# Wells-Group/pmg-dolfinx

Hardware: NVIDIA B200
Metric: fine-level Gdof/s per p-MG V-cycle (P4->P2->P1, Chebyshev(2), CSR coarse solve) (higher is better)
Workload: dtype f64

## Files before the change

### include/pmgx.h

```cpp
#ifndef PMGX_H
#define PMGX_H

#include <stddef.h>
#include <stdint.h>

#ifdef __cplusplus
extern "C" {
#endif

#define PMGX_OK 0
#define PMGX_ERR_ARG 1
#define PMGX_ERR_CUDA 2
#define PMGX_ERR_NCCL 3
#define PMGX_ERR_NUMERIC 4
#define PMGX_ERR_UNSUPPORTED 5

#define PMGX_MAX_DEGREE 8
#define PMGX_NCCL_ID_BYTES 128

typedef struct pmgx_ctx pmgx_ctx;
typedef struct pmgx_halo pmgx_halo;
typedef struct pmgx_operator pmgx_operator;
typedef struct pmgx_cheb pmgx_cheb;
typedef struct pmgx_cg pmgx_cg;
typedef struct pmgx_interp pmgx_interp;
typedef struct pmgx_coarse pmgx_coarse;
typedef struct pmgx_vcycle pmgx_vcycle;
typedef struct pmgx_boxmesh pmgx_boxmesh;
typedef struct pmgx_ghostmesh pmgx_ghostmesh;
typedef struct pmgx_amg_hier pmgx_amg_hier;

const char* pmgx_last_error_string(void);
int pmgx_version(void);

int pmgx_gll_tables(int degree, double* points_h, double* weights_h, double* dphi_h);
int pmgx_gll_interp_1d(int degree_coarse, int degree_fine, double* interp_h);

int pmgx_tqli(double* d_h, double* e_h, int n);

int pmgx_nccl_unique_id(void* id_h);
int pmgx_ctx_create(int device, int rank, int nranks, const void* nccl_id_h, pmgx_ctx** out);
int pmgx_ctx_destroy(pmgx_ctx* ctx);
int pmgx_ctx_sync(pmgx_ctx* ctx);
void* pmgx_ctx_stream(pmgx_ctx* ctx);
int pmgx_ctx_rank(pmgx_ctx* ctx);
int pmgx_ctx_nranks(pmgx_ctx* ctx);
long long pmgx_ctx_launch_count(pmgx_ctx* ctx);
int pmgx_ctx_uses_p2p(pmgx_ctx* ctx);
int pmgx_ctx_profile(pmgx_ctx* ctx, int on);
int pmgx_ctx_profile_read(pmgx_ctx* ctx, int degree, double* ms_total_h, long long* launches_h);

int pmgx_halo_create(pmgx_ctx* ctx, int n_owned, int n_ghost,
                     int n_send_nbr, const int* send_ranks_h, const int* send_offsets_h,
                     const int32_t* send_idx_h,
                     int n_recv_nbr, const int* recv_ranks_h, const int* recv_offsets_h,
                     const int32_t* recv_idx_h, pmgx_halo** out);
int pmgx_halo_destroy(pmgx_halo* h);
int pmgx_halo_uses_p2p(pmgx_halo* h);
int pmgx_halo_fwd_begin(pmgx_halo* h, double* x);
int pmgx_halo_fwd_end(pmgx_halo* h, double* x);
int pmgx_halo_rev(pmgx_halo* h, double* x);
int pmgx_pack(pmgx_ctx* ctx, int n, const int32_t* idx, const double* in, double* out);
int pmgx_unpack(pmgx_ctx* ctx, int n, const int32_t* idx, const double* in, double* out);
int pmgx_unpack_add(pmgx_ctx* ctx, int n, const int32_t* idx, const double* in, double* out);

int pmgx_vec_set(pmgx_ctx* ctx, double* x, long long n, double v);
int pmgx_vec_copy(pmgx_ctx* ctx, double* a, const double* b, long long n);
int pmgx_vec_axpy(pmgx_ctx* ctx, double* r, double alpha, const double* x,
                  const double* y, long long n);
int pmgx_vec_scale(pmgx_ctx* ctx, double* r, double alpha, long long n);
int pmgx_vec_pointwise_mult(pmgx_ctx* ctx, double* w, const double* x,
                            const double* y, long long n);
int pmgx_vec_mask_bc(pmgx_ctx* ctx, double* b, const int8_t* bc, long long n);
int pmgx_vec_dot(pmgx_ctx* ctx, const double* a, const double* b, long long n, double* result_h);
int pmgx_vec_norm(pmgx_ctx* ctx, const double* a, long long n, int linf, double* result_h);

#define PMGX_LAP_DEFAULT 0
#define PMGX_LAP_LITERAL_DETJ 1
#define PMGX_LAP_NO_DIAG 2
#define PMGX_LAP_STREAM_G 4
#define PMGX_LAP_RECOMPUTE_G 8
#define PMGX_LAP_GEOM_Q2 16

int pmgx_laplacian_create(pmgx_ctx* ctx, int degree, int n_cells, const int32_t* dofmap,
                          const double* xgeom, int n_points, const int32_t* geom_dofmap,
                          const double* kappa, const int32_t* lcells_h, int n_lcells,
                          const int32_t* bcells_h, int n_bcells, const int8_t* bc_marker,
                          int n_owned, int n_ghost, pmgx_halo* halo, int flags,
                          pmgx_operator** out);
int pmgx_laplacian_get_G(pmgx_operator* op, double* G_out);
int pmgx_laplacian_is_affine(pmgx_operator* op);
int pmgx_laplacian_kernel_name(pmgx_operator* op, char* name_h, int cap);
int pmgx_laplacian_device_bytes(pmgx_operator* op, long long* bytes_h);

int pmgx_csr_create(pmgx_ctx* ctx, int n_rows, int n_ghost, const int32_t* row_ptr_h,
                    const int32_t* off_diag_offset_h, const int32_t* cols_h,
                    const double* values_h, pmgx_halo* halo, pmgx_operator** out);
int pmgx_csr_from_laplacian(pmgx_operator* lap, pmgx_operator** out);
long long pmgx_csr_nnz(pmgx_operator* op);
int pmgx_csr_get(pmgx_operator* op, int32_t* row_ptr_h, int32_t* cols_h, double* values_h);

int pmgx_operator_apply(pmgx_operator* op, double* x, double* y);
int pmgx_operator_get_diag_inverse(pmgx_operator* op, double* out);
int pmgx_operator_set_diag_inverse(pmgx_operator* op, const double* in);
int pmgx_operator_n_owned(pmgx_operator* op);
int pmgx_operator_n_ghost(pmgx_operator* op);
int pmgx_operator_destroy(pmgx_operator* op);

int pmgx_cheb_create(pmgx_ctx* ctx, int n_owned, int n_ghost, double eig_min, double eig_max,
                     pmgx_cheb** out);
int pmgx_cheb_set_max_iterations(pmgx_cheb* s, int max_iter);
int pmgx_cheb_solve(pmgx_cheb* s, pmgx_operator* A, double* x, const double* b,
                    double* resid_hist_h);
int pmgx_cheb_residual(pmgx_cheb* s, pmgx_operator* A, double* x, const double* b,
                       double* rnorm_h);
int pmgx_cheb_destroy(pmgx_cheb* s);

int pmgx_cg_create(pmgx_ctx* ctx, int n_owned, int n_ghost, pmgx_cg** out);
int pmgx_cg_set_max_iterations(pmgx_cg* s, int max_iter);
int pmgx_cg_set_tolerance(pmgx_cg* s, double rtol);
int pmgx_cg_store_coefficients(pmgx_cg* s, int on);
int pmgx_cg_set_preconditioner(pmgx_cg* s, pmgx_vcycle* M);
int pmgx_cg_solve(pmgx_cg* s, pmgx_operator* A, double* x, const double* b, int* iters_h);
int pmgx_cg_num_coefficients(pmgx_cg* s);
int pmgx_cg_get_coefficients(pmgx_cg* s, double* alphas_h, double* betas_h, double* residuals_h);
int pmgx_cg_get_history(pmgx_cg* s, double* rnorm0_h, double* rnorms_h, int* n_h);
int pmgx_cg_compute_eigenvalues(pmgx_cg* s, double* eig_h);
int pmgx_cg_destroy(pmgx_cg* s);

int pmgx_interp_create(pmgx_ctx* ctx, int degree_coarse, int degree_fine, int n_cells,
                       const int32_t* dofmap_coarse, const int32_t* dofmap_fine,
                       int n_coarse_total, int n_fine_total,
                       const int32_t* lcells_h, int n_lcells, const int32_t* bcells_h,
                       int n_bcells, pmgx_halo* halo_c, pmgx_halo* halo_f, pmgx_interp** out);
int pmgx_interp_prolong(pmgx_interp* it, double* coarse, double* fine);
int pmgx_interp_restrict(pmgx_interp* it, double* fine, double* coarse);
int pmgx_interp_destroy(pmgx_interp* it);

int pmgx_coarse_create(pmgx_ctx* ctx, pmgx_operator* A_csr, int max_iter, double rtol,
                       pmgx_coarse** out);
int pmgx_coarse_create_amg(pmgx_ctx* ctx, pmgx_operator* A_csr, int max_iter, double rtol, int nu,
                           int min_coarse, int max_levels, pmgx_coarse** out);
int pmgx_coarse_solve(pmgx_coarse* cs, double* x, const double* b, int* iters_h);
int pmgx_coarse_last_iterations(pmgx_coarse* cs);
int pmgx_coarse_last_status(pmgx_coarse* cs, int* converged_h, double* rel_residual_h);
int pmgx_coarse_num_levels(pmgx_coarse* cs);
int pmgx_coarse_level_info(pmgx_coarse* cs, int level, long long* out_h);
int pmgx_coarse_apply_preconditioner(pmgx_coarse* cs, const double* r, double* u);
int pmgx_coarse_destroy(pmgx_coarse* cs);

typedef int (*pmgx_allgather_fn)(void* user, const void* mine, size_t bytes, void* all);
int pmgx_amg_setup_h(int n_rows, const int32_t* row_ptr_h, const int32_t* cols_h, const double* values_h,
                     int min_coarse, int max_levels, pmgx_amg_hier** out);
int pmgx_amg_setup_dist_h(int rank, int nranks, int n_owned, int n_ghost, const int32_t* row_ptr_h,
                          const int32_t* cols_h, const double* values_h, int n_send_nbr, const int* send_ranks_h,
                          const int* send_offsets_h, const int32_t* send_idx_h, int n_recv_nbr,
                          const int* recv_ranks_h, const int* recv_offsets_h, const int32_t* recv_idx_h,
                          pmgx_allgather_fn allgather, void* user, int min_coarse, int max_levels,
                          pmgx_amg_hier** out);
int pmgx_amg_level_dist_sizes(pmgx_amg_hier* h, int level, long long* out_h);
int pmgx_amg_level_get_restriction(pmgx_amg_hier* h, int level, int32_t* r_ptr_h, int32_t* r_cols_h, double* r_vals_h);
int pmgx_amg_level_dist_get(pmgx_amg_hier* h, int level, int* ghost_src_h, int32_t* ghost_rid_h, int* send_ranks_h,
                            int* send_offsets_h, int32_t* send_idx_h, int* recv_ranks_h, int* recv_offsets_h,
                            int32_t* recv_idx_h, double* inv_rows_h);
int pmgx_csr_drop_zeros_h(int n_rows, const int32_t* ptr_h, const int32_t* cols_h, const double* vals_h,
                          int32_t* out_ptr_h, int32_t* out_cols_h, double* out_vals_h, long long* kept_h);
int pmgx_amg_num_levels(pmgx_amg_hier* h);
int pmgx_amg_level_sizes(pmgx_amg_hier* h, int level, long long* out_h);
int pmgx_amg_level_get(pmgx_amg_hier* h, int level, int32_t* a_ptr_h, int32_t* a_cols_h, double* a_vals_h,
                       int32_t* p_ptr_h, int32_t* p_cols_h, double* p_vals_h, double* lmax_h);
int pmgx_amg_destroy(pmgx_amg_hier* h);

#define PMGX_VC_DEFAULT 0
#define PMGX_VC_LITERAL_REFERENCE_BC 1
#define PMGX_VC_DIAGNOSTICS 2
#define PMGX_VC_LITERAL_SEQUENCE 4
int pmgx_vcycle_create(pmgx_ctx* ctx, int n_levels, pmgx_operator** ops, pmgx_cheb** smoothers,
                       pmgx_interp** interps, const int8_t** bc_markers, pmgx_coarse* coarse,
                       int flags, pmgx_vcycle** out);
int pmgx_vcycle_apply(pmgx_vcycle* vc, const double* b, double* u, double* rnorm_h);
int pmgx_vcycle_get_diagnostics(pmgx_vcycle* vc, double* out_h, int cap, int* n_h);
int pmgx_vcycle_destroy(pmgx_vcycle* vc);

int pmgx_boxmesh_create(int nx, int ny, int nz, int px, int py, int pz, int rank,
                        double perturb, uint64_t seed, pmgx_boxmesh** out);
int pmgx_boxmesh_destroy(pmgx_boxmesh* m);
int pmgx_boxmesh_sizes(pmgx_boxmesh* m, long long* out_h);
int pmgx_boxmesh_geometry(pmgx_boxmesh* m, double* xgeom_h, int32_t* geom_dofmap_h);
int pmgx_boxmesh_cell_lists(pmgx_boxmesh* m, int32_t* lcells_h, int32_t* bcells_h);
int pmgx_boxmesh_space_sizes(pmgx_boxmesh* m, int degree, long long* out_h);
int pmgx_boxmesh_space(pmgx_boxmesh* m, int degree, int32_t* dofmap_h, int8_t* bc_h,
                       long long* l2g_h, double* coords_h);
int pmgx_boxmesh_halo_lists(pmgx_boxmesh* m, int degree, int* send_ranks_h, int* send_offsets_h,
                            int32_t* send_idx_h, int* recv_ranks_h, int* recv_offsets_h,
                            int32_t* recv_idx_h);
int pmgx_boxmesh_fit(long long ndofs_total, int order, int* nxyz_h);

int pmgx_ghostmesh_create(int rank, int nranks, long long n_cells, const long long* cell_vertices_h,
                          const int* cell_owner_h, long long n_vertices, const double* coords_h,
                          pmgx_ghostmesh** out);
int pmgx_ghostmesh_create_q2(int rank, int nranks, long long n_cells, const long long* cell_nodes_h,
                             const int* cell_owner_h, long long n_nodes, const double* coords_h,
                             pmgx_ghostmesh** out);
int pmgx_ghostmesh_nodes_per_cell(pmgx_ghostmesh* m);
int pmgx_ghostmesh_destroy(pmgx_ghostmesh* m);
int pmgx_ghostmesh_sizes(pmgx_ghostmesh* m, long long* out_h);
int pmgx_ghostmesh_geometry(pmgx_ghostmesh* m, double* xgeom_h, int32_t* geom_dofmap_h, long long* cell_gid_h);
int pmgx_ghostmesh_cell_lists(pmgx_ghostmesh* m, int32_t* lcells_h, int32_t* bcells_h);
int pmgx_ghostmesh_space_sizes(pmgx_ghostmesh* m, int degree, long long* out_h);
int pmgx_ghostmesh_space(pmgx_ghostmesh* m, int degree, int32_t* dofmap_h, int8_t* bc_h, long long* l2g_h,
                         double* coords_h);
int pmgx_ghostmesh_halo_lists(pmgx_ghostmesh* m, int degree, int* send_ranks_h, int* send_offsets_h,
                              int32_t* send_idx_h, int* recv_ranks_h, int* recv_offsets_h, int32_t* recv_idx_h);

int pmgx_laplacian_rhs(pmgx_operator* lap, const double* fvals, double g, double* b);
int pmgx_bc_marker_exterior(pmgx_ctx* ctx, int degree, int n_cells, const int32_t* geom_dofmap,
                            const int32_t* dofmap, int n_owned, int n_ghost, pmgx_halo* halo, int8_t* marker_out);

int pmgx_laplacian_lift(pmgx_operator* lap, const double* gvals, double* b);

#ifdef __cplusplus
}
#endif
#endif
```

### pmg_dolfinx_b200/api.py

```python
import ctypes
import numpy as np
import torch

from .capi import lib, check, ptr, PmgxError


LAP_DEFAULT = 0
LAP_LITERAL_DETJ = 1
LAP_NO_DIAG = 2
LAP_STREAM_G = 4
LAP_RECOMPUTE_G = 8
LAP_GEOM_Q2 = 16

Q2_CORNERS = (0, 2, 6, 8, 18, 20, 24, 26)


def corner_columns(geometry_dofmap):
    g = geometry_dofmap.reshape(-1, 27)[:, list(Q2_CORNERS)]
    return g.contiguous() if isinstance(g, torch.Tensor) else np.ascontiguousarray(g)


def _np(a, dtype):
    return np.ascontiguousarray(a, dtype=dtype)


class Context:

    def __init__(self, device=0, rank=0, nranks=1, nccl_id=None):
        h = ctypes.c_void_p()
        idp = None
        if nccl_id is not None:
            self._id = (ctypes.c_char * 128).from_buffer_copy(bytes(nccl_id))
            idp = ctypes.addressof(self._id)
        check(lib.pmgx_ctx_create(device, rank, nranks, idp, ctypes.addressof(h)))
        self.h = h
        self.device = torch.device("cuda", device)
        self.rank, self.nranks = rank, nranks
        self.stream = torch.cuda.ExternalStream(lib.pmgx_ctx_stream(self.h), device=self.device)
        torch.cuda.set_device(self.device)
        torch.cuda.set_stream(self.stream)

    @staticmethod
    def nccl_unique_id():
        buf = (ctypes.c_char * 128)()
        check(lib.pmgx_nccl_unique_id(ctypes.addressof(buf)))
        return bytes(buf)

    def sync(self):
        check(lib.pmgx_ctx_sync(self.h))

    def launch_count(self):
        return int(lib.pmgx_ctx_launch_count(self.h))

    def zeros(self, n, dtype=torch.float64):
        return torch.zeros(int(n), dtype=dtype, device=self.device)

    def to_device(self, a, dtype=None):
        t = torch.as_tensor(np.ascontiguousarray(a))
        if dtype is not None:
            t = t.to(dtype)
        return t.to(self.device)

    def close(self):
        if self.h:
            check(lib.pmgx_ctx_destroy(self.h))
            self.h = None


def gll_tables(degree):
    n = degree + 1
    x, w, D = np.zeros(n), np.zeros(n), np.zeros(n * n)
    check(lib.pmgx_gll_tables(degree, ptr(x), ptr(w), ptr(D)))
    return x, w, D.reshape(n, n)


def gll_interp_1d(pc, pf):
    M = np.zeros((pf + 1) * (pc + 1))
    check(lib.pmgx_gll_interp_1d(pc, pf, ptr(M)))
    return M.reshape(pf + 1, pc + 1)


def exterior_bc_marker(ctx, degree, geometry_dofmap, dofmap, n_owned, n_ghost=0, halo=None):
    out = torch.zeros(int(n_owned) + int(n_ghost), dtype=torch.int8, device=ctx.device)
    n_cells = int(geometry_dofmap.numel() // 8)
    check(lib.pmgx_bc_marker_exterior(ctx.h, degree, n_cells, ptr(geometry_dofmap), ptr(dofmap), int(n_owned), int(n_ghost),
                                      halo.h if halo is not None else None, ptr(out)))
    return out


def tqli(d, e):
    d = _np(d, np.float64).copy()
    e = _np(e, np.float64).copy()
    check(lib.pmgx_tqli(ptr(d), ptr(e), len(d)))
    return d


def boxmesh_fit(ndofs_total, order):
    out = np.zeros(3, dtype=np.int32)
    check(lib.pmgx_boxmesh_fit(int(ndofs_total), order, ptr(out)))
    return tuple(int(v) for v in out)


class BoxMesh:

    def __init__(self, n, pgrid=(1, 1, 1), rank=0, perturb=0.0, seed=1234):
        h = ctypes.c_void_p()
        check(lib.pmgx_boxmesh_create(n[0], n[1], n[2], pgrid[0], pgrid[1], pgrid[2], rank,
                                      float(perturb), seed, ctypes.addressof(h)))
        self.h = h
        self.n, self.pgrid, self.rank = tuple(n), tuple(pgrid), rank
        s = np.zeros(5, dtype=np.int64)
        check(lib.pmgx_boxmesh_sizes(self.h, ptr(s)))
        self.n_cells, self.n_owned_cells, self.n_points, nl, nb = (int(v) for v in s)
        self.xgeom = np.zeros((self.n_points, 3))
        self.geom_dofmap = np.zeros((self.n_cells, 8), dtype=np.int32)
        check(lib.pmgx_boxmesh_geometry(self.h, ptr(self.xgeom), ptr(self.geom_dofmap)))
        self.lcells = np.zeros(nl, dtype=np.int32)
        self.bcells = np.zeros(nb, dtype=np.int32)
        check(lib.pmgx_boxmesh_cell_lists(self.h, ptr(self.lcells), ptr(self.bcells)))

    def space(self, degree, want_coords=False):
        s = np.zeros(7, dtype=np.int64)
        check(lib.pmgx_boxmesh_space_sizes(self.h, degree, ptr(s)))
        sp = HostSpace()
        sp.degree = degree
        (sp.n_owned, sp.n_ghost, nsn, nst, nrn, nrt, sp.n_global) = (int(v) for v in s)
        nd3 = (degree + 1) ** 3
        nt = sp.n_owned + sp.n_ghost
        sp.dofmap = np.zeros((self.n_cells, nd3), dtype=np.int32)
        sp.bc = np.zeros(nt, dtype=np.int8)
        sp.l2g = np.zeros(nt, dtype=np.int64)
        sp.coords = np.zeros((nt, 3)) if want_coords else None
        check(lib.pmgx_boxmesh_space(self.h, degree, ptr(sp.dofmap), ptr(sp.bc), ptr(sp.l2g),
                                     ptr(sp.coords)))
        sp.send_ranks = np.zeros(nsn, dtype=np.int32)
        sp.send_offsets = np.zeros(nsn + 1, dtype=np.int32)
        sp.send_idx = np.zeros(nst, dtype=np.int32)
        sp.recv_ranks = np.zeros(nrn, dtype=np.int32)
        sp.recv_offsets = np.zeros(nrn + 1, dtype=np.int32)
        sp.recv_idx = np.zeros(nrt, dtype=np.int32)
        check(lib.pmgx_boxmesh_halo_lists(self.h, degree, ptr(sp.send_ranks), ptr(sp.send_offsets),
                                          ptr(sp.send_idx), ptr(sp.recv_ranks), ptr(sp.recv_offsets),
                                          ptr(sp.recv_idx)))
        return sp

    def close(self):
        if self.h:
            lib.pmgx_boxmesh_destroy(self.h)
            self.h = None


class HostSpace:
    pass


class GhostLayerMesh:

    def __init__(self, cell_vertices, cell_owner, coords, rank=0, nranks=1):
        cv = _np(cell_vertices, np.int64)
        npc = 27 if cv.ndim == 2 and cv.shape[1] == 27 else 8
        cv = cv.reshape(-1, npc)
        ow = _np(cell_owner, np.int32)
        xs = _np(coords, np.float64).reshape(-1, 3)
        h = ctypes.c_void_p()
        create = lib.pmgx_ghostmesh_create_q2 if npc == 27 else lib.pmgx_ghostmesh_create
        check(create(rank, nranks, len(cv), ptr(cv), ptr(ow), len(xs), ptr(xs), ctypes.addressof(h)))
        self.h, self.rank, self.nranks = h, rank, nranks
        self.nodes_per_cell = int(lib.pmgx_ghostmesh_nodes_per_cell(self.h))
        s = np.zeros(5, dtype=np.int64)
        check(lib.pmgx_ghostmesh_sizes(self.h, ptr(s)))
        self.n_cells, self.n_owned_cells, self.n_points, nl, nb = (int(v) for v in s)
        self.xgeom = np.zeros((self.n_points, 3))
        self.geom_dofmap = np.zeros((self.n_cells, self.nodes_per_cell), dtype=np.int32)
        self.cell_gid = np.zeros(self.n_cells, dtype=np.int64)
        check(lib.pmgx_ghostmesh_geometry(self.h, ptr(self.xgeom), ptr(self.geom_dofmap), ptr(self.cell_gid)))
        self.lcells = np.zeros(nl, dtype=np.int32)
        self.bcells = np.zeros(nb, dtype=np.int32)
        check(lib.pmgx_ghostmesh_cell_lists(self.h, ptr(self.lcells), ptr(self.bcells)))

    def space(self, degree, want_coords=True):
        s = np.zeros(7, dtype=np.int64)
        check(lib.pmgx_ghostmesh_space_sizes(self.h, degree, ptr(s)))
        sp = HostSpace()
        sp.degree = degree
        (sp.n_owned, sp.n_ghost, nsn, nst, nrn, nrt, sp.n_global) = (int(v) for v in s)
        nt = sp.n_owned + sp.n_ghost
        sp.dofmap = np.zeros((self.n_cells, (degree + 1) ** 3), dtype=np.int32)
        sp.bc = np.zeros(nt, dtype=np.int8)
        sp.l2g = np.zeros(nt, dtype=np.int64)
        sp.coords = np.zeros((nt, 3)) if want_coords else None
        check(lib.pmgx_ghostmesh_space(self.h, degree, ptr(sp.dofmap), ptr(sp.bc), ptr(sp.l2g), ptr(sp.coords)))
        sp.send_ranks = np.zeros(nsn, dtype=np.int32)
        sp.send_offsets = np.zeros(nsn + 1, dtype=np.int32)
        sp.send_idx = np.zeros(nst, dtype=np.int32)
        sp.recv_ranks = np.zeros(nrn, dtype=np.int32)
        sp.recv_offsets = np.zeros(nrn + 1, dtype=np.int32)
        sp.recv_idx = np.zeros(nrt, dtype=np.int32)
        check(lib.pmgx_ghostmesh_halo_lists(self.h, degree, ptr(sp.send_ranks), ptr(sp.send_offsets), ptr(sp.send_idx),
                                            ptr(sp.recv_ranks), ptr(sp.recv_offsets), ptr(sp.recv_idx)))
        return sp

    def close(self):
        if self.h:
            lib.pmgx_ghostmesh_destroy(self.h)
            self.h = None


class Halo:

    def __init__(self, ctx, n_owned, n_ghost, send_ranks=(), send_offsets=(0,), send_idx=(),
                 recv_ranks=(), recv_offsets=(0,), recv_idx=()):
        self.ctx, self.n_owned, self.n_ghost = ctx, int(n_owned), int(n_ghost)
        sr, so, si = _np(send_ranks, np.int32), _np(send_offsets, np.int32), _np(send_idx, np.int32)
        rr, ro, ri = _np(recv_ranks, np.int32), _np(recv_offsets, np.int32), _np(recv_idx, np.int32)
        h = ctypes.c_void_p()
        check(lib.pmgx_halo_create(ctx.h, self.n_owned, self.n_ghost, len(sr), ptr(sr), ptr(so), ptr(si),
                                   len(rr), ptr(rr), ptr(ro), ptr(ri), ctypes.addressof(h)))
        self.h = h

    @classmethod
    def from_space(cls, ctx, sp):
        return cls(ctx, sp.n_owned, sp.n_ghost, sp.send_ranks, sp.send_offsets, sp.send_idx,
                   sp.recv_ranks, sp.recv_offsets, sp.recv_idx)


class Vector:

    def __init__(self, ctx, n_owned, n_ghost=0, halo=None):
        self.ctx, self.n_owned, self.n_ghost, self.halo = ctx, int(n_owned), int(n_ghost), halo
        self.data = ctx.zeros(self.n_owned + self.n_ghost)

    @property
    def size_local(self):
        return self.n_owned

    def set(self, v):
        check(lib.pmgx_vec_set(self.ctx.h, ptr(self.data), self.n_owned + self.n_ghost, float(v)))

    def copy_from_host(self, a):
        a = _np(a, np.float64)
        self.data[: self.n_owned].copy_(torch.from_numpy(a[: self.n_owned]))

    def array(self):
        return self.data

    def mutable_array(self):
        return self.data

    def data_copy(self):
        self.ctx.sync()
        return self.data.cpu().numpy()

    def scatter_fwd_begin(self):
        if self.halo is not None:
            check(lib.pmgx_halo_fwd_begin(self.halo.h, ptr(self.data)))

    def scatter_fwd_end(self):
        if self.halo is not None:
            check(lib.pmgx_halo_fwd_end(self.halo.h, ptr(self.data)))

    def scatter_fwd(self):
        self.scatter_fwd_begin()
        self.scatter_fwd_end()

    def scatter_rev(self):
        if self.halo is not None:
            check(lib.pmgx_halo_rev(self.halo.h, ptr(self.data)))


def _same(a, b):
    if a.n_owned != b.n_owned:
        raise PmgxError(1, "Incompatible vector sizes")


def inner_product(a, b):
    _same(a, b)
    r = ctypes.c_double()
    check(lib.pmgx_vec_dot(a.ctx.h, ptr(a.data), ptr(b.data), a.n_owned, ctypes.addressof(r)))
    return r.value


def squared_norm(a):
    return inner_product(a, a)


def norm(a, kind="l2"):
    if kind not in ("l2", "linf"):
        raise PmgxError(1, "Norm type not supported")
    r = ctypes.c_double()
    check(lib.pmgx_vec_norm(a.ctx.h, ptr(a.data), a.n_owned, 1 if kind == "linf" else 0, ctypes.addressof(r)))
    return r.value


def axpy(r, alpha, x, y):
    check(lib.pmgx_vec_axpy(r.ctx.h, ptr(r.data), float(alpha), ptr(x.data), ptr(y.data), x.n_owned))


def scale(r, alpha):
    check(lib.pmgx_vec_scale(r.ctx.h, ptr(r.data), float(alpha), r.n_owned + r.n_ghost))


def copy(a, b):
    check(lib.pmgx_vec_copy(a.ctx.h, ptr(a.data), ptr(b.data), a.n_owned))


def pointwise_mult(w, x, y):
    check(lib.pmgx_vec_pointwise_mult(w.ctx.h, ptr(w.data), ptr(x.data), ptr(y.data), x.n_owned))


class _Operator:
    h = None

    def __call__(self, x, y):
        check(lib.pmgx_operator_apply(self.h, ptr(x.data), ptr(y.data)))

    def get_diag_inverse(self, v):
        check(lib.pmgx_operator_get_diag_inverse(self.h, ptr(v.data)))

    def set_diag_inverse(self, v):
        check(lib.pmgx_operator_set_diag_inverse(self.h, ptr(v.data)))

    @property
    def n_owned(self):
        return lib.pmgx_operator_n_owned(self.h)

    @property
    def n_ghost(self):
        return lib.pmgx_operator_n_ghost(self.h)

    def destroy(self):
        if self.h:
            check(lib.pmgx_operator_destroy(self.h))
            self.h = None


class MatFreeLaplacian(_Operator):

    def __init__(self, ctx, degree, coefficients, dofmap, xgeom, geometry_dofmap, lcells, bcells,
                 bc_marker, n_owned, n_ghost=0, halo=None, flags=0):
        self.ctx, self.degree = ctx, degree
        self._keep = (coefficients, dofmap, xgeom, geometry_dofmap, bc_marker, halo)
        lc, bc_ = _np(lcells, np.int32), _np(bcells, np.int32)
        n_cells = int(dofmap.numel() // ((degree + 1) ** 3)) if degree >= 0 else 0
        h = ctypes.c_void_p()
        check(lib.pmgx_laplacian_create(
            ctx.h, degree, n_cells, ptr(dofmap), ptr(xgeom), int(xgeom.numel() // 3), ptr(geometry_dofmap),
            ptr(coefficients), ptr(lc), len(lc), ptr(bc_), len(bc_), ptr(bc_marker), int(n_owned),
            int(n_ghost), halo.h if halo is not None else None, flags, ctypes.addressof(h)))
        self.h = h
        self.n_list = len(lc) + len(bc_)

    def is_affine(self):
        return bool(lib.pmgx_laplacian_is_affine(self.h))

    def device_bytes(self):
        b = ctypes.c_longlong()
        check(lib.pmgx_laplacian_device_bytes(self.h, ctypes.addressof(b)))
        return b.value

    def kernel_name(self):
        buf = ctypes.create_string_buffer(96)
        check(lib.pmgx_laplacian_kernel_name(self.h, ctypes.addressof(buf), 96))
        return buf.value.decode()

    def geometry_factors(self):
        nq = (self.degree + 1) ** 3
        G = self.ctx.zeros(self.n_list * nq * 6)
        check(lib.pmgx_laplacian_get_G(self.h, ptr(G)))
        self.ctx.sync()
        return G.cpu().numpy().reshape(self.n_list, nq, 6)

    def assemble_rhs(self, fvals, g, b):
        check(lib.pmgx_laplacian_rhs(self.h, ptr(fvals), float(g), ptr(b.data)))

    def lift(self, gvals, b):
        check(lib.pmgx_laplacian_lift(self.h, ptr(gvals), ptr(b.data)))

    def to_csr(self):
        return MatrixOperator._from_handle(self.ctx, lambda out: lib.pmgx_csr_from_laplacian(self.h, out))


class MatrixOperator(_Operator):

    def __init__(self, ctx, row_ptr, off_diag_offset, cols, values, n_ghost=0, halo=None):
        self.ctx = ctx
        rp, od = _np(row_ptr, np.int32), _np(off_diag_offset, np.int32)
        co, va = _np(cols, np.int32), _np(values, np.float64)
        h = ctypes.c_void_p()
        check(lib.pmgx_csr_create(ctx.h, len(rp) - 1, int(n_ghost), ptr(rp), ptr(od), ptr(co), ptr(va),
                                  halo.h if halo is not None else None, ctypes.addressof(h)))
        self.h = h

    @classmethod
    def _from_handle(cls, ctx, make):
        self = cls.__new__(cls)
        self.ctx = ctx
        h = ctypes.c_void_p()
        check(make(ctypes.addressof(h)))
        self.h = h
        return self

    def nnz(self):
        return int(lib.pmgx_csr_nnz(self.h))

    def to_host(self):
        n = self.n_owned
        rp = np.zeros(n + 1, dtype=np.int32)
        co = np.zeros(self.nnz(), dtype=np.int32)
        va = np.zeros(self.nnz())
        check(lib.pmgx_csr_get(self.h, ptr(rp), ptr(co), ptr(va)))
        return rp, co, va


class Chebyshev:

    def __init__(self, ctx, n_owned, n_ghost, eig_range):
        self.ctx = ctx
        h = ctypes.c_void_p()
        check(lib.pmgx_cheb_create(ctx.h, int(n_owned), int(n_ghost), float(eig_range[0]), float(eig_range[1]),
                                   ctypes.addressof(h)))
        self.h = h
        self.max_iter = 0

    def set_max_iterations(self, n):
        self.max_iter = int(n)
        check(lib.pmgx_cheb_set_max_iterations(self.h, int(n)))

    def solve(self, A, x, b, verbose=False):
        hist = np.zeros(self.max_iter + 1) if verbose else None
        check(lib.pmgx_cheb_solve(self.h, A.h, ptr(x.data), ptr(b.data), ptr(hist)))
        return hist

    def residual(self, A, x, b):
        r = ctypes.c_double()
        check(lib.pmgx_cheb_residual(self.h, A.h, ptr(x.data), ptr(b.data), ctypes.addressof(r)))
        return r.value


class CGSolver:

    def __init__(self, ctx, n_owned, n_ghost=0):
        self.ctx = ctx
        h = ctypes.c_void_p()
        check(lib.pmgx_cg_create(ctx.h, int(n_owned), int(n_ghost), ctypes.addressof(h)))
        self.h = h

    def set_max_iterations(self, n):
        check(lib.pmgx_cg_set_max_iterations(self.h, int(n)))

    def set_tolerance(self, rtol):
        check(lib.pmgx_cg_set_tolerance(self.h, float(rtol)))

    def store_coefficients(self, on):
        check(lib.pmgx_cg_store_coefficients(self.h, 1 if on else 0))

    def set_preconditioner(self, pmg):
        if pmg is not None and pmg.h is None:
            pmg._build()
        self._pmg = pmg
        check(lib.pmgx_cg_set_preconditioner(self.h, pmg.h if pmg is not None else None))

    def solve(self, A, x, b, verbose=False):
        k = ctypes.c_int()
        check(lib.pmgx_cg_solve(self.h, A.h, ptr(x.data), ptr(b.data), ctypes.addressof(k)))
        return k.value

    def _coeffs(self):
        n = lib.pmgx_cg_num_coefficients(self.h)
        a, b, r = np.zeros(n), np.zeros(n), np.zeros(n)
        check(lib.pmgx_cg_get_coefficients(self.h, ptr(a), ptr(b), ptr(r)))
        return a, b, r

    def alphas(self):
        return self._coeffs()[0]

    def betas(self):
        return self._coeffs()[1]

    def residual(self):
        return self._coeffs()[2][-1]

    def history(self, cap=4096):
        r0, n = ctypes.c_double(), ctypes.c_int()
        h = np.zeros(cap)
        check(lib.pmgx_cg_get_history(self.h, ctypes.addressof(r0), ptr(h), ctypes.addressof(n)))
        return r0.value, h[: n.value].copy()

    def compute_eigenvalues(self):
        n = lib.pmgx_cg_num_coefficients(self.h)
        e = np.zeros(max(n, 1))
        check(lib.pmgx_cg_compute_eigenvalues(self.h, ptr(e)))
        return e[:n]


class Interpolator:

    def __init__(self, ctx, degree_coarse, degree_fine, Q1_dofmap, Q2_dofmap, n_coarse_total, n_fine_total,
                 l_cells, b_cells, halo_coarse=None, halo_fine=None):
        self.ctx = ctx
        self._keep = (Q1_dofmap, Q2_dofmap, halo_coarse, halo_fine)
        lc, bc_ = _np(l_cells, np.int32), _np(b_cells, np.int32)
        n_cells = int(Q1_dofmap.numel() // ((degree_coarse + 1) ** 3))
        h = ctypes.c_void_p()
        check(lib.pmgx_interp_create(ctx.h, degree_coarse, degree_fine, n_cells, ptr(Q1_dofmap), ptr(Q2_dofmap),
                                     int(n_coarse_total), int(n_fine_total), ptr(lc), len(lc), ptr(bc_), len(bc_),
                                     halo_coarse.h if halo_coarse is not None else None,
                                     halo_fine.h if halo_fine is not None else None, ctypes.addressof(h)))
        self.h = h

    def interpolate(self, Q1_vector, Q2_vector):
        check(lib.pmgx_interp_prolong(self.h, ptr(Q1_vector.data), ptr(Q2_vector.data)))

    def reverse_interpolate(self, Q2_vector, Q1_vector):
        check(lib.pmgx_interp_restrict(self.h, ptr(Q2_vector.data), ptr(Q1_vector.data)))


class CoarseSolverType:

    def __init__(self, ctx, A_csr, max_iter=60, rtol=1e-5, amg=True, nu=2, min_coarse=0, max_levels=0):
        self.ctx, self.A, self.amg = ctx, A_csr, bool(amg)
        h = ctypes.c_void_p()
        if amg:
            check(lib.pmgx_coarse_create_amg(ctx.h, A_csr.h, int(max_iter), float(rtol), int(nu), int(min_coarse),
                                             int(max_levels), ctypes.addressof(h)))
        else:
            check(lib.pmgx_coarse_create(ctx.h, A_csr.h, int(max_iter), float(rtol), ctypes.addressof(h)))
        self.h = h

    def solve(self, x, b):
        k = ctypes.c_int()
        check(lib.pmgx_coarse_solve(self.h, ptr(x.data), ptr(b.data), ctypes.addressof(k)))
        return k.value

    def last_iterations(self):
        return int(lib.pmgx_coarse_last_iterations(self.h))

    def last_status(self):
        c, r = ctypes.c_int(), ctypes.c_double()
        check(lib.pmgx_coarse_last_status(self.h, ctypes.addressof(c), ctypes.addressof(r)))
        return bool(c.value), r.value

    def levels(self):
        out = []
        for l in range(lib.pmgx_coarse_num_levels(self.h)):
            v = np.zeros(5, dtype=np.int64)
            check(lib.pmgx_coarse_level_info(self.h, l, ptr(v)))
            out.append(tuple(int(t) for t in v))
        return out

    def apply_preconditioner(self, r, u):
        check(lib.pmgx_coarse_apply_preconditioner(self.h, ptr(r.data), ptr(u.data)))


class MultigridPreconditioner:

    def __init__(self, ctx, bc_markers, flags=0):
        self.ctx, self.bc_markers, self.flags = ctx, list(bc_markers), flags
        self.solvers = self.operators = self.interpolators = None
        self.coarse_solver = None
        self.h = None

    def set_solvers(self, s):
        self.solvers = list(s)

    def set_coarse_solver(self, s):
        self.coarse_solver = s

    def set_operators(self, o):
        self.operators = list(o)

    def set_interpolators(self, i):
        self.interpolators = list(i)

    def _build(self):
        nl = len(self.operators)
        P = ctypes.c_void_p * nl
        ops = P(*[o.h for o in self.operators])
        sm = P(*[s.h for s in self.solvers])
        bcs = P(*[ptr(b) for b in self.bc_markers])
        its = (ctypes.c_void_p * max(nl - 1, 1))(*[i.h for i in (self.interpolators or [])])
        h = ctypes.c_void_p()
        check(lib.pmgx_vcycle_create(self.ctx.h, nl, ctypes.addressof(ops), ctypes.addressof(sm),
                                     ctypes.addressof(its), ctypes.addressof(bcs),
                                     self.coarse_solver.h if self.coarse_solver is not None else None,
                                     self.flags, ctypes.addressof(h)))
        self.h = h

    def apply(self, x, y, verbose=False):
        if self.h is None:
            self._build()
        r = ctypes.c_double()
        check(lib.pmgx_vcycle_apply(self.h, ptr(x.data), ptr(y.data), ctypes.addressof(r) if verbose else None))
        return r.value if verbose else None

    def diagnostics(self, cap=256):
        out, n = np.zeros(cap), ctypes.c_int()
        check(lib.pmgx_vcycle_get_diagnostics(self.h, ptr(out), cap, ctypes.addressof(n)))
        return out[: n.value].copy()
```

### pmg_dolfinx_b200/csrc/amg.cu

```cuda
#include "common.hpp"
#include "operator.hpp"
#include "csr.hpp"
#include "solvers.hpp"
#include "amg.hpp"

#include <algorithm>
#include <cstdlib>
#include <cstring>

namespace pmgx
{
namespace
{
__global__ void __launch_bounds__(256)
k_dense_rows(int n_rows, int n_cols, const double* __restrict__ inv, const double* __restrict__ b,
             double* __restrict__ x)
{
  const int row = (blockIdx.x * blockDim.x + threadIdx.x) >> 5, lane = threadIdx.x & 31;
  if (row >= n_rows)
    return;
  const double* r = inv + (size_t)row * n_cols;
  double s = 0.0;
  for (int c = lane; c < n_cols; c += 32)
    s = fma(r[c], b[c], s);
#pragma unroll
  for (int o = 16; o > 0; o >>= 1)
    s += __shfl_xor_sync(0xffffffffu, s, o);
  if (lane == 0)
    x[row] = s;
}

__global__ void k_permute(int n, const int32_t* __restrict__ perm, const double* __restrict__ in, double* __restrict__ out)
{
  const int g = blockIdx.x * blockDim.x + threadIdx.x;
  if (g < n)
    out[g] = in[perm[g]];
}

struct RectSell
{
  int n_rows = 0;
  DevBuf<long long> slice_ptr;
  DevBuf<int32_t> cols;
  DevBuf<double> vals;
  void upload(const amg::Csr& M, cudaStream_t st)
  {
    n_rows = M.n_rows;
    const int ns = (n_rows + 31) / 32;
    std::vector<long long> sp((size_t)ns + 1, 0);
    for (int s = 0; s < ns; ++s)
    {
      int w = 0;
      for (int r = s * 32; r < std::min(n_rows, s * 32 + 32); ++r)
        w = std::max(w, (int)(M.ptr[r + 1] - M.ptr[r]));
      sp[s + 1] = sp[s] + (long long)w * 32;
    }
    std::vector<int32_t> c((size_t)std::max<long long>(sp[ns], 1), 0);
    std::vector<double> v((size_t)std::max<long long>(sp[ns], 1), 0.0);
    for (int r = 0; r < n_rows; ++r)
      for (int32_t j = M.ptr[r], k = 0; j < M.ptr[r + 1]; ++j, ++k)
      {
        const size_t p = (size_t)sp[r >> 5] + (size_t)k * 32 + (r & 31);
        c[p] = M.cols[j];
        v[p] = M.vals[j];
      }
    slice_ptr.upload(sp.data(), sp.size(), st);
    cols.upload(c.data(), c.size(), st);
    vals.upload(v.data(), v.size(), st);
  }
};

struct RectCsr
{
  int n_rows = 0;
  DevBuf<int32_t> ptr, cols;
  DevBuf<double> vals;
  void upload(const amg::Csr& M, cudaStream_t st)
  {
    n_rows = M.n_rows;
    ptr.upload(M.ptr.data(), M.ptr.size(), st);
    cols.upload(M.cols.data(), M.cols.size(), st);
    vals.upload(M.vals.data(), M.vals.size(), st);
  }
};

pmgx_halo* make_halo(pmgx_ctx* c, int n_owned, int n_ghost, const amg::Plan& p)
{
  if (c->nranks == 1)
    return nullptr;
  pmgx_halo* h = nullptr;
  const int rc = pmgx_halo_create(c, n_owned, n_ghost, (int)p.send_ranks.size(), p.send_ranks.data(), p.send_offsets.data(),
                                  p.send_idx.data(), (int)p.recv_ranks.size(), p.recv_ranks.data(), p.recv_offsets.data(),
                                  p.recv_idx.data(), &h);
  if (rc != PMGX_OK)
    throw Error{rc};
  static const bool ss = !(getenv("PMGX_AMG_SINGLE_STREAM") && atoi(getenv("PMGX_AMG_SINGLE_STREAM")) == 0);
  h->single_stream = ss && h->p2p && h->n_send() + h->n_recv() <= 65536;
  return h;
}

struct AmgPrecond : Precond
{
  struct Lv
  {
    int n_owned = 0, n_ghost = 0;
    long long nnz = 0;
    pmgx_operator* A = nullptr;
    bool own_A = false;
    pmgx_operator* A_lp = nullptr;
    pmgx_halo* halo = nullptr;
    pmgx_halo* halo_v = nullptr;
    pmgx_cheb* sm = nullptr;
    RectCsr R;
    RectSell P;
    DevBuf<double> x, b;
    DevBuf<double> x2, r2;
    long long nnz_p = 0;
    bool dense = false;
    int n_global = 0;
    DevBuf<double> inv;
    pmgx_halo* gather = nullptr;
    bool repl_first = false;
    int n_mine = 0;
    pmgx_halo* repl_gather = nullptr;
    DevBuf<double> bg;
    DevBuf<int32_t> perm;
  };
  pmgx_ctx* ctx = nullptr;
  std::vector<Lv> lv;
  int nu = 2;
  int gamma = 1;
  int gamma_from = 0;

  ~AmgPrecond() override
  {
    for (Lv& L : lv)
    {
      if (L.sm)
        pmgx_cheb_destroy(L.sm);
      if (L.A_lp)
        pmgx_operator_destroy(L.A_lp);
      if (L.own_A && L.A)
        pmgx_operator_destroy(L.A);
      if (L.halo)
        pmgx_halo_destroy(L.halo);
      if (L.gather)
        pmgx_halo_destroy(L.gather);
      if (L.repl_gather)
        pmgx_halo_destroy(L.repl_gather);
    }
  }

  void cycle(int l, const double* b, double* x)
  {
    Lv& L = lv[l];
    if (l + 1 == (int)lv.size())
    {
      if (L.dense)
      {
        double* bb = L.b.p;
        if (b != bb)
          vec::copy(ctx, bb, b, L.n_owned);
        if (L.gather)
        {
          halo_fwd_begin(L.gather, bb);
          halo_fwd_end(L.gather, bb);
        }
        if (L.n_owned > 0)
        {
          k_dense_rows<<<(L.n_owned * 32 + 255) / 256, 256, 0, ctx->stream>>>(L.n_owned, L.n_global, L.inv.p, bb, x);
          check_launch("k_dense_rows");
          count_launch(ctx);
        }
      }
      else
        cheb_solve(L.sm, L.A, x, b, nullptr, true, CHEB_R_NONE);
      return;
    }
    Lv& C = lv[l + 1];
    pmgx_operator* As = L.A_lp ? L.A_lp : L.A;
    cheb_solve(L.sm, As, x, b, nullptr, true, CHEB_R_FULL);
    if (L.halo_v)
    {
      halo_fwd_begin(L.halo_v, L.sm->r.p);
      halo_fwd_end(L.halo_v, L.sm->r.p);
    }
    if (C.repl_first)
    {
      spmv_rect(ctx, C.n_mine, L.R.ptr.p, L.R.cols.p, L.R.vals.p, L.sm->r.p, C.bg.p, false, 32);
      halo_fwd_begin(C.repl_gather, C.bg.p);
      halo_fwd_end(C.repl_gather, C.bg.p);
      k_permute<<<(C.n_owned + 255) / 256, 256, 0, ctx->stream>>>(C.n_owned, C.perm.p, C.bg.p, C.b.p);
      check_launch("k_permute");
      count_launch(ctx);
    }
    else
      spmv_rect(ctx, C.n_owned, L.R.ptr.p, L.R.cols.p, L.R.vals.p, L.sm->r.p, C.b.p, false, 32);
    cycle(l + 1, C.b.p, C.x.p);
    if (gamma == 2 && l >= gamma_from && l + 2 < (int)lv.size())
    {
      C.A->apply(C.x.p, C.r2.p);
      vec::axpy(ctx, C.r2.p, -1.0, C.r2.p, C.b.p, C.n_owned);
      cycle(l + 1, C.r2.p, C.x2.p);
      vec::axpy(ctx, C.x.p, 1.0, C.x2.p, C.x.p, C.n_owned);
    }
    if (C.halo_v)
    {
      halo_fwd_begin(C.halo_v, C.x.p);
      halo_fwd_end(C.halo_v, C.x.p);
    }
    spmv_sell_rect(ctx, L.n_owned, L.P.slice_ptr.p, L.P.cols.p, L.P.vals.p, C.x.p, x, true);
    cheb_solve(L.sm, As, x, b, nullptr, false, CHEB_R_NONE);
  }

  void apply(const double* r, double* u) override { cycle(0, r, u); }
};

amg::Plan plan_of(pmgx_halo* h)
{
  amg::Plan p;
  if (!h)
    return p;
  p.send_ranks = h->send_ranks;
  p.send_offsets = h->send_offsets;
  p.recv_ranks = h->recv_ranks;
  p.recv_offsets = h->recv_offsets;
  if (p.send_offsets.empty())
    p.send_offsets.assign(1, 0);
  if (p.recv_offsets.empty())
    p.recv_offsets.assign(1, 0);
  p.send_idx.resize((size_t)h->n_send());
  p.recv_idx.resize((size_t)h->n_recv());
  if (!p.send_idx.empty())
    PMGX_CUDA(cudaMemcpy(p.send_idx.data(), h->send_idx.p, p.send_idx.size() * sizeof(int32_t), cudaMemcpyDeviceToHost));
  if (!p.recv_idx.empty())
    PMGX_CUDA(cudaMemcpy(p.recv_idx.data(), h->recv_idx.p, p.recv_idx.size() * sizeof(int32_t), cudaMemcpyDeviceToHost));
  return p;
}
}
}

using pmgx::AmgPrecond;

extern "C"
{
int pmgx_coarse_create_amg(pmgx_ctx* ctx, pmgx_operator* A, int max_iter, double rtol, int nu, int min_coarse,
                           int max_levels, pmgx_coarse** out)
{
  PMGX_API_BEGIN
  PMGX_REQUIRE(ctx && A && out && max_iter >= 0, "coarse_create_amg: bad arguments");
  PMGX_REQUIRE(A->kind == pmgx_operator::CSR, "coarse_create_amg: the operator must be an assembled CSR operator");
  PMGX_REQUIRE(nu >= 1 && nu <= 8, "coarse_create_amg: nu must be in 1..8");
  PMGX_CUDA(cudaSetDevice(ctx->device));
  if (min_coarse <= 0)
    min_coarse = 600;
  if (max_levels <= 0)
    max_levels = 12;
  auto* Ac = static_cast<pmgx::CsrOperator*>(A);
  PMGX_REQUIRE(ctx->nranks == 1 || Ac->halo || Ac->n_ghost == 0, "coarse_create_amg: the operator has ghosts but no halo");
  pmgx::amg::Csr A0;
  A0.ptr.resize((size_t)Ac->n_owned + 1);
  A0.cols.resize((size_t)Ac->nnz);
  A0.vals.resize((size_t)Ac->nnz);
  {
    const int rc = pmgx_csr_get(A, A0.ptr.data(), A0.cols.data(), A0.vals.data());
    if (rc != PMGX_OK)
      return rc;
    std::vector<std::pair<int32_t, double>> row;
    for (int i = 0; i < Ac->n_owned; ++i)
    {
      bool sorted = true;
      for (int32_t j = A0.ptr[i] + 1; j < A0.ptr[i + 1] && sorted; ++j)
        sorted = A0.cols[j - 1] < A0.cols[j];
      if (sorted)
        continue;
      row.clear();
      for (int32_t j = A0.ptr[i]; j < A0.ptr[i + 1]; ++j)
        row.emplace_back(A0.cols[j], A0.vals[j]);
      std::sort(row.begin(), row.end());
      for (size_t t = 0; t < row.size(); ++t)
        A0.cols[A0.ptr[i] + t] = row[t].first, A0.vals[A0.ptr[i] + t] = row[t].second;
    }
  }
  pmgx::amg::Csr Az;
  if (Ac->n_owned > 0)
  {
    A0.n_rows = Ac->n_owned;
    A0.n_cols = Ac->n_owned + Ac->n_ghost;
    Az = pmgx::amg::drop_stored_zeros(A0);
    if (Az.nnz() * 5 > A0.nnz() * 4)
      Az = pmgx::amg::Csr();
  }
  const pmgx::amg::Plan plan0 = pmgx::plan_of(Ac->halo);
  pmgx::amg::Comm cm;
  cm.rank = ctx->rank;
  cm.nranks = ctx->nranks;
  cm.allgather = [ctx](const void* mine, size_t bytes, void* all)
  {
    std::vector<char> buf;
    pmgx::p2p::allgather_bytes(ctx, mine, bytes, buf);
    std::memcpy(all, buf.data(), bytes * (size_t)ctx->nranks);
  };
  pmgx::amg::Hierarchy H;
  pmgx::amg::setup(H, std::move(A0), Ac->n_owned, Ac->n_ghost, plan0, cm, min_coarse, max_levels);

  std::unique_ptr<AmgPrecond> M(new AmgPrecond());
  M->ctx = ctx;
  M->nu = nu;
  int nu_coarse = nu;
  if (const char* e = getenv("PMGX_AMG_NU_COARSE"))
    nu_coarse = std::min(std::max(atoi(e), 1), 8);
  if (const char* e = getenv("PMGX_AMG_GAMMA"))
    M->gamma = atoi(e) == 2 ? 2 : 1;
  if (const char* e = getenv("PMGX_AMG_GAMMA_FROM"))
    M->gamma_from = std::max(atoi(e), 0);
  const bool use_lp = !(getenv("PMGX_AMG_LP") && atoi(getenv("PMGX_AMG_LP")) == 0);
  const int fuse_from = getenv("PMGX_AMG_FUSE_FROM") ? atoi(getenv("PMGX_AMG_FUSE_FROM")) : 0;
  const int nl = (int)H.levels.size();
  M->lv.resize((size_t)nl);
  for (int l = 0; l < nl; ++l)
  {
    pmgx::amg::Level& L = H.levels[l];
    AmgPrecond::Lv& D = M->lv[l];
    D.n_owned = L.n_owned;
    D.n_ghost = L.n_ghost;
    D.nnz = L.A.nnz();
    const bool last = l + 1 == nl;
    if (l == 0)
    {
      D.A = A;
      D.halo_v = Ac->halo;
      if (!Az.ptr.empty())
      {
        std::vector<int32_t> off((size_t)Ac->n_owned);
        for (int i = 0; i < Ac->n_owned; ++i)
        {
          int32_t j = Az.ptr[i];
          while (j < Az.ptr[i + 1] && Az.cols[j] < Ac->n_owned)
            ++j;
          off[i] = j;
        }
        pmgx_operator* Acmp = nullptr;
        const int rc = pmgx_csr_create(ctx, Ac->n_owned, Ac->n_ghost, Az.ptr.data(), off.data(), Az.cols.data(),
                                       Az.vals.data(), Ac->halo, &Acmp);
        if (rc != PMGX_OK)
          return rc;
        D.A = Acmp;
        D.own_A = true;
      }
    }
    else
    {
      if (!L.replicated)
      {
        D.halo = pmgx::make_halo(ctx, L.n_owned, L.n_ghost, L.plan);
        D.halo_v = D.halo;
      }
      else if (L.n_mine > 0 || !L.gather_perm.empty())
      {
        D.repl_first = true;
        D.n_mine = L.n_mine;
        D.repl_gather = pmgx::make_halo(ctx, L.n_mine, L.n_owned - L.n_mine, L.repl_plan);
        D.bg.alloc((size_t)std::max(L.n_owned, 1));
        PMGX_CUDA(cudaMemsetAsync(D.bg.p, 0, (size_t)std::max(L.n_owned, 1) * sizeof(double), ctx->stream));
        D.perm.upload(L.gather_perm.data(), L.gather_perm.size(), ctx->stream);
      }
      std::vector<int32_t> off((size_t)L.n_owned);
      for (int i = 0; i < L.n_owned; ++i)
      {
        int32_t j = L.A.ptr[i];
        while (j < L.A.ptr[i + 1] && L.A.cols[j] < L.n_owned)
          ++j;
        off[i] = j;
      }
      const int rc = pmgx_csr_create(ctx, L.n_owned, L.n_ghost, L.A.ptr.data(), off.data(), L.A.cols.data(),
                                     L.A.vals.data(), D.halo, &D.A);
      if (rc != PMGX_OK)
        return rc;
      D.own_A = true;
      const size_t nt = (size_t)L.n_owned + L.n_ghost;
      for (auto* buf : {&D.x, &D.b, &D.x2, &D.r2})
      {
        buf->alloc(nt);
        if (nt > 0)
          PMGX_CUDA(cudaMemsetAsync(buf->p, 0, nt * sizeof(double), ctx->stream));
      }
    }
    {
      const int rc = pmgx_cheb_create(ctx, L.n_owned, L.n_ghost, 0.1 * L.lmax, L.lmax, &D.sm);
      if (rc != PMGX_OK)
        return rc;
      D.sm->max_iter = (last && !L.dense) ? 4 * nu : (l == 0 ? nu : nu_coarse);
      D.sm->fuse = l >= fuse_from;
    }
    if (l == 0 && !last && use_lp)
      D.A_lp = pmgx::make_lp(static_cast<pmgx::CsrOperator*>(D.A));
    D.nnz_p = L.P.nnz();
    if (!last)
    {
      D.P.upload(pmgx::amg::drop_stored_zeros(L.P), ctx->stream);
      D.R.upload(pmgx::amg::drop_stored_zeros(L.R), ctx->stream);
    }
    else if (L.dense)
    {
      D.dense = true;
      D.n_global = (int)L.n_global;
      D.inv.upload(L.inv_rows.data(), L.inv_rows.size(), ctx->stream);
      const int n_gather = (int)L.n_global - L.n_owned;
      if (!L.replicated)
        D.gather = pmgx::make_halo(ctx, L.n_owned, n_gather, L.gather_plan);
      const size_t nt = (size_t)L.n_owned + std::max(L.n_ghost, n_gather);
      D.b.alloc(nt);
      if (nt > 0)
        PMGX_CUDA(cudaMemsetAsync(D.b.p, 0, nt * sizeof(double), ctx->stream));
    }
  }
  PMGX_CUDA(cudaStreamSynchronize(ctx->stream));

  pmgx_coarse* cs = nullptr;
  const int rc = pmgx_coarse_create(ctx, M->lv[0].A, max_iter, rtol, &cs);
  if (rc != PMGX_OK)
    return rc;
  cs->M = M.release();
  cs->check_every = 1;
  if (const char* e = getenv("PMGX_COARSE_CHECK_EVERY"))
    cs->check_every = std::max(atoi(e), 1);
  *out = cs;
  PMGX_API_END
}

int pmgx_coarse_num_levels(pmgx_coarse* cs)
{
  if (!cs)
    return -1;
  return cs->M ? (int)static_cast<AmgPrecond*>(cs->M)->lv.size() : 1;
}

int pmgx_coarse_level_info(pmgx_coarse* cs, int level, long long* out_h)
{
  PMGX_API_BEGIN
  PMGX_REQUIRE(cs && out_h && level >= 0 && level < pmgx_coarse_num_levels(cs), "coarse_level_info: bad arguments");
  if (!cs->M)
  {
    out_h[0] = cs->A->n_owned;
    out_h[1] = pmgx_csr_nnz(cs->A);
    out_h[2] = cs->A->n_ghost;
    out_h[3] = 0;
    out_h[4] = 0;
  }
  else
  {
    const AmgPrecond::Lv& L = static_cast<AmgPrecond*>(cs->M)->lv[level];
    out_h[0] = L.n_owned;
    out_h[1] = L.nnz;
    out_h[2] = L.n_ghost;
    out_h[3] = L.dense ? 1 : 0;
    out_h[4] = L.nnz_p;
  }
  PMGX_API_END
}

int pmgx_coarse_apply_preconditioner(pmgx_coarse* cs, const double* r, double* u)
{
  PMGX_API_BEGIN
  PMGX_REQUIRE(cs && r && u && r != u, "coarse_apply_preconditioner: bad arguments");
  PMGX_CUDA(cudaSetDevice(cs->ctx->device));
  if (cs->M)
    cs->M->apply(r, u);
  else
    pmgx::vec::pointwise_mult(cs->ctx, u, r, cs->A->diag_inv.p, cs->A->n_owned);
  PMGX_API_END
}
}
```

### pmg_dolfinx_b200/csrc/common.hpp

```cpp
#pragma once

#include <cuda_runtime.h>
#include <nccl.h>

#include <cstdarg>
#include <cstdint>
#include <cstdio>
#include <memory>
#include <algorithm>
#include <stdexcept>
#include <string>
#include <utility>
#include <vector>

#include "../../include/pmgx.h"

namespace pmgx
{
void set_error(const char* fmt, ...);

struct Error
{
  int code;
};

#define PMGX_CUDA(call)                                                                            \
  do                                                                                               \
  {                                                                                                \
    cudaError_t _e = (call);                                                                       \
    if (_e != cudaSuccess)                                                                         \
    {                                                                                              \
      pmgx::set_error("%s:%d CUDA error: %s (%s)", __FILE__, __LINE__, cudaGetErrorString(_e),     \
                      #call);                                                                      \
      throw pmgx::Error{PMGX_ERR_CUDA};                                                            \
    }                                                                                              \
  } while (0)

#define PMGX_NCCL(call)                                                                            \
  do                                                                                               \
  {                                                                                                \
    ncclResult_t _e = (call);                                                                      \
    if (_e != ncclSuccess)                                                                         \
    {                                                                                              \
      pmgx::set_error("%s:%d NCCL error: %s (%s)", __FILE__, __LINE__, ncclGetErrorString(_e),     \
                      #call);                                                                      \
      throw pmgx::Error{PMGX_ERR_NCCL};                                                            \
    }                                                                                              \
  } while (0)

#define PMGX_REQUIRE(cond, ...)                                                                    \
  do                                                                                               \
  {                                                                                                \
    if (!(cond))                                                                                   \
    {                                                                                              \
      pmgx::set_error(__VA_ARGS__);                                                                \
      throw pmgx::Error{PMGX_ERR_ARG};                                                             \
    }                                                                                              \
  } while (0)

#define PMGX_API_BEGIN try {
#define PMGX_API_END                                                                               \
  }                                                                                                \
  catch (const pmgx::Error& e) { return e.code; }                                                  \
  catch (const std::exception& e)                                                                  \
  {                                                                                                \
    pmgx::set_error("exception: %s", e.what());                                                    \
    return PMGX_ERR_ARG;                                                                           \
  }                                                                                                \
  return PMGX_OK;

template <typename T>
struct DevBuf
{
  T* p = nullptr;
  size_t n = 0;
  DevBuf() = default;
  DevBuf(const DevBuf&) = delete;
  DevBuf& operator=(const DevBuf&) = delete;
  DevBuf(DevBuf&& o) noexcept : p(o.p), n(o.n)
  {
    o.p = nullptr;
    o.n = 0;
  }
  ~DevBuf() { release(); }
  void alloc(size_t count)
  {
    release();
    n = count;
    if (count > 0)
      PMGX_CUDA(cudaMalloc(&p, count * sizeof(T)));
  }
  void release()
  {
    if (p)
      cudaFree(p);
    p = nullptr;
    n = 0;
  }
  void upload(const T* h, size_t count, cudaStream_t s)
  {
    alloc(count);
    if (count > 0)
    {
      PMGX_CUDA(cudaMemcpyAsync(p, h, count * sizeof(T), cudaMemcpyHostToDevice, s));
      PMGX_CUDA(cudaStreamSynchronize(s));
    }
  }
};
}

struct pmgx_ctx
{
  int device = 0;
  int rank = 0;
  int nranks = 1;
  int num_sms = 148;
  cudaStream_t stream = nullptr;
  cudaStream_t comm_stream = nullptr;
  ncclComm_t comm = nullptr;
  double* d_scalars = nullptr;
  double* h_scalars = nullptr;
  double* h_scalars_dev = nullptr;
  unsigned int* d_counter = nullptr;
  double* d_partials = nullptr;
  int max_red_blocks = 0;
  bool p2p = false;
  double* ar_local = nullptr;
  double** d_ar_peers = nullptr;
  std::vector<void*> p2p_mapped;
  unsigned long long* d_ar_epoch = nullptr;
  unsigned long long p2p_timeout_ns = 600ull * 1000000000ull;
  long long launches = 0;
  bool profiling = false;
  std::vector<std::pair<cudaEvent_t, cudaEvent_t>> prof[PMGX_MAX_DEGREE + 1];
};

namespace pmgx
{
inline void count_launch(pmgx_ctx* ctx, int n = 1) { ctx->launches += n; }
inline void check_launch(const char* what)
{
  cudaError_t e = cudaGetLastError();
  if (e != cudaSuccess)
  {
    set_error("kernel launch failed (%s): %s", what, cudaGetErrorString(e));
    throw Error{PMGX_ERR_CUDA};
  }
}

void gll_points_weights(int n, std::vector<double>& x, std::vector<double>& w);
void gll_deriv_matrix(const std::vector<double>& x, std::vector<double>& D);
void gll_interp_matrix(int pc, int pf, std::vector<double>& M);

namespace p2p
{
void allgather_bytes(pmgx_ctx* c, const void* mine, size_t bytes, std::vector<char>& all);
bool all_agree(pmgx_ctx* c, bool mine);
void ctx_setup(pmgx_ctx* c);
void ctx_teardown(pmgx_ctx* c);
void allreduce(pmgx_ctx* c, int slot, int count, bool is_max);
}

namespace vec
{
void set(pmgx_ctx* c, double* x, long long n, double v);
void copy(pmgx_ctx* c, double* a, const double* b, long long n);
void axpy(pmgx_ctx* c, double* r, double alpha, const double* x, const double* y, long long n);
void scale(pmgx_ctx* c, double* r, double alpha, long long n);
void pointwise_mult(pmgx_ctx* c, double* w, const double* x, const double* y, long long n);
void mask_bc(pmgx_ctx* c, double* b, const int8_t* bc, long long n);
void allreduce_scalars(pmgx_ctx* c, int slot, int count, bool is_max);
void dot_device(pmgx_ctx* c, const double* a, const double* b, long long n, int slot);
double read_scalar(pmgx_ctx* c, int slot);
void publish_scalars(pmgx_ctx* c, int slot, int count);
double dot(pmgx_ctx* c, const double* a, const double* b, long long n);
double norm_linf(pmgx_ctx* c, const double* a, long long n);
}
}
```

### pmg_dolfinx_b200/csrc/csr.cu

```cuda
#include "common.hpp"
#include "operator.hpp"
#include "csr.hpp"
#include "solvers.hpp"

namespace pmgx
{
namespace
{
constexpr int LPR = 8;
constexpr int ST = 256;

constexpr int UNR = 4;
template <bool ACCUM>
__global__ void __launch_bounds__(ST)
k_spmv(int n_rows, const double* __restrict__ vals, const int32_t* __restrict__ beg,
       const int32_t* __restrict__ end, const int32_t* __restrict__ cols,
       const double* __restrict__ x, double* __restrict__ y)
{
  const int gt = blockIdx.x * blockDim.x + threadIdx.x;
  const int row = gt / LPR, lane = gt % LPR;
  double s = 0.0;
  if (row < n_rows)
  {
    const int e = end[row];
    for (int j0 = beg[row] + lane; j0 < e; j0 += UNR * LPR)
    {
      int c[UNR];
      double v[UNR];
#pragma unroll
      for (int t = 0; t < UNR; ++t)
      {
        const int jj = j0 + t * LPR;
        const bool ok = jj < e;
        c[t] = ok ? __ldcs(cols + jj) : -1;
        v[t] = ok ? __ldcs(vals + jj) : 0.0;
      }
#pragma unroll
      for (int t = 0; t < UNR; ++t)
        if (c[t] >= 0)
          s = fma(v[t], x[c[t]], s);
    }
  }
#pragma unroll
  for (int o = LPR / 2; o > 0; o >>= 1)
    s += __shfl_xor_sync(0xffffffffu, s, o);
  if (row < n_rows && lane == 0)
    y[row] = ACCUM ? y[row] + s : s;
}

__global__ void __launch_bounds__(ST)
k_spmv_ghost_rows(int n_list, const int32_t* __restrict__ rows, const double* __restrict__ vals,
                  const int32_t* __restrict__ off_diag, const int32_t* __restrict__ row_ptr,
                  const int32_t* __restrict__ cols, const double* __restrict__ x, double* __restrict__ y)
{
  const int gt = blockIdx.x * blockDim.x + threadIdx.x;
  const int li = gt / LPR, lane = gt % LPR;
  double s = 0.0;
  int row = -1;
  if (li < n_list)
  {
    row = rows[li];
    const int e = row_ptr[row + 1];
    for (int j = off_diag[row] + lane; j < e; j += LPR)
      s = fma(vals[j], x[cols[j]], s);
  }
#pragma unroll
  for (int o = LPR / 2; o > 0; o >>= 1)
    s += __shfl_xor_sync(0xffffffffu, s, o);
  if (row >= 0 && lane == 0)
    y[row] += s;
}

template <int MODE>
__device__ __forceinline__ void cheb_row(int i, double q, const double* __restrict__ in, const ChebEp& e)
{
  if (MODE == ChebEp::INIT)
  {
    const double rv = q * (-1.0) + e.b[i];
    e.r[i] = rv;
    e.z_out[i] = (rv * e.dinv[i]) * e.c0;
  }
  else if (MODE == ChebEp::LAST)
    e.r[i] = q * (-1.0) + e.r[i];
  else
  {
    const double rv = q * (-1.0) + e.r[i];
    const double zo = in[i];
    const double zs = zo * e.c1;
    const double zv = (rv * e.dinv[i]) * e.c2 + zs;
    if (MODE == ChebEp::STEP)
    {
      e.r[i] = rv;
      e.z_out[i] = zv;
    }
    const double xo = e.defer == 2 ? zo : (e.defer == 1 ? zo * 1.0 + e.x[i] : e.x[i]);
    e.x[i] = zv * 1.0 + xo;
  }
}

template <typename VT, bool D16, int MODE>
__global__ void __launch_bounds__(ST)
k_spmv_cheb(int n_rows, const VT* __restrict__ vals, const int32_t* __restrict__ beg, const int32_t* __restrict__ end,
            const int32_t* __restrict__ row_ptr, const int16_t* __restrict__ dcol, const int32_t* __restrict__ cols,
            const double* __restrict__ x, const ChebEp e)
{
  const int gt = blockIdx.x * blockDim.x + threadIdx.x;
  const int row = gt / LPR, lane = gt % LPR;
  double s = 0.0;
  if (row < n_rows)
  {
    const int en = end[row];
    for (int j0 = beg[row] + lane; j0 < en; j0 += UNR * LPR)
    {
      int c[UNR];
      VT v[UNR];
#pragma unroll
      for (int t = 0; t < UNR; ++t)
      {
        const int jj = j0 + t * LPR;
        const bool ok = jj < en;
        c[t] = ok ? (D16 ? row + (int)__ldcs(dcol + jj) : __ldcs(cols + jj)) : -1;
        v[t] = ok ? __ldcs(vals + jj) : VT(0);
      }
#pragma unroll
      for (int t = 0; t < UNR; ++t)
        if (c[t] >= 0)
          s = fma((double)v[t], x[c[t]], s);
    }
  }
#pragma unroll
  for (int o = LPR / 2; o > 0; o >>= 1)
    s += __shfl_xor_sync(0xffffffffu, s, o);
  __shared__ double sq[ST / LPR];
  if (lane == 0)
    sq[threadIdx.x / LPR] = s;
  __syncthreads();
  if (threadIdx.x < ST / LPR)
  {
    const int r = blockIdx.x * (ST / LPR) + threadIdx.x;
    if (r < n_rows)
    {
      if (end[r] < row_ptr[r + 1])
        e.scratch[r] = sq[threadIdx.x];
      else
        cheb_row<MODE>(r, sq[threadIdx.x], x, e);
    }
  }
}

template <int MODE>
__global__ void __launch_bounds__(ST)
k_spmv_cheb_ghost_rows(int n_list, const int32_t* __restrict__ rows, const double* __restrict__ vals,
                       const int32_t* __restrict__ off_diag, const int32_t* __restrict__ row_ptr,
                       const int32_t* __restrict__ cols, const double* __restrict__ x, const ChebEp e)
{
  const int gt = blockIdx.x * blockDim.x + threadIdx.x;
  const int li = gt / LPR, lane = gt % LPR;
  double s = 0.0;
  int row = -1;
  if (li < n_list)
  {
    row = rows[li];
    const int en = row_ptr[row + 1];
    for (int j = off_diag[row] + lane; j < en; j += LPR)
      s = fma(vals[j], x[cols[j]], s);
  }
#pragma unroll
  for (int o = LPR / 2; o > 0; o >>= 1)
    s += __shfl_xor_sync(0xffffffffu, s, o);
  if (row >= 0 && lane == 0)
    cheb_row<MODE>(row, e.scratch[row] + s, x, e);
}

template <typename VT, bool D16>
void launch_spmv_cheb(pmgx_ctx* c, int grid, int n_rows, const VT* vals, const int32_t* beg, const int32_t* end,
                      const int32_t* row_ptr, const int16_t* dcol, const int32_t* cols, const double* x, const ChebEp& e)
{
  switch (e.mode)
  {
  case ChebEp::INIT: k_spmv_cheb<VT, D16, ChebEp::INIT><<<grid, ST, 0, c->stream>>>(n_rows, vals, beg, end, row_ptr, dcol, cols, x, e); break;
  case ChebEp::STEP: k_spmv_cheb<VT, D16, ChebEp::STEP><<<grid, ST, 0, c->stream>>>(n_rows, vals, beg, end, row_ptr, dcol, cols, x, e); break;
  case ChebEp::LAST: k_spmv_cheb<VT, D16, ChebEp::LAST><<<grid, ST, 0, c->stream>>>(n_rows, vals, beg, end, row_ptr, dcol, cols, x, e); break;
  default: k_spmv_cheb<VT, D16, ChebEp::XONLY><<<grid, ST, 0, c->stream>>>(n_rows, vals, beg, end, row_ptr, dcol, cols, x, e); break;
  }
  check_launch("k_spmv_cheb");
  count_launch(c);
}

void launch_ghost_rows_cheb(const CsrOperator* A, const double* x, const ChebEp& e)
{
  pmgx_ctx* c = A->ctx;
  const int g2 = (int)(((long long)A->n_ghost_rows * LPR + ST - 1) / ST);
#define PMGX_GR(M)                                                                                                     \
  k_spmv_cheb_ghost_rows<M><<<g2, ST, 0, c->stream>>>(A->n_ghost_rows, A->ghost_rows.p, A->values.p, A->off_diag.p,    \
                                                      A->row_ptr.p, A->cols.p, x, e)
  switch (e.mode)
  {
  case ChebEp::INIT: PMGX_GR(ChebEp::INIT); break;
  case ChebEp::STEP: PMGX_GR(ChebEp::STEP); break;
  case ChebEp::LAST: PMGX_GR(ChebEp::LAST); break;
  default: PMGX_GR(ChebEp::XONLY); break;
  }
#undef PMGX_GR
  check_launch("k_spmv_cheb_ghost_rows");
  count_launch(c);
}

__global__ void k_flag_ghost_rows(int n_rows, const int32_t* __restrict__ off_diag,
                                  const int32_t* __restrict__ row_ptr, int32_t* __restrict__ count,
                                  int32_t* __restrict__ list)
{
  const int i = blockIdx.x * blockDim.x + threadIdx.x;
  if (i < n_rows && off_diag[i] < row_ptr[i + 1])
    list[atomicAdd(count, 1)] = i;
}

__global__ void k_extract_diag_inv(int n_rows, const double* __restrict__ vals,
                                   const int32_t* __restrict__ row_ptr,
                                   const int32_t* __restrict__ cols, double* __restrict__ dinv)
{
  const int i = blockIdx.x * blockDim.x + threadIdx.x;
  if (i >= n_rows)
    return;
  double d = 0.0;
  for (int j = row_ptr[i]; j < row_ptr[i + 1]; ++j)
    if (cols[j] == i)
      d = 1.0 / vals[j];
  dinv[i] = d;
}

constexpr int SLICE = 32;

template <bool D16>
__device__ __forceinline__ double sell_row(int row, int n_rows, const long long* __restrict__ slice_ptr,
                                           const float* __restrict__ vals, const int16_t* __restrict__ dcol,
                                           const int32_t* __restrict__ cols, const double* __restrict__ x)
{
  const int s = row >> 5, lane = row & 31;
  const long long b = slice_ptr[s];
  const int w = (int)((slice_ptr[s + 1] - b) >> 5);
  const float* v = vals + b + lane;
  const int16_t* d = dcol + b + lane;
  const int32_t* c = cols + b + lane;
  const int r = row < n_rows ? row : n_rows - 1;
  double s0 = 0.0, s1 = 0.0;
  int k = 0;
  for (; k + 4 <= w; k += 4)
  {
    float vv[4];
    int cc[4];
#pragma unroll
    for (int t = 0; t < 4; ++t)
    {
      vv[t] = __ldcs(v + (k + t) * SLICE);
      cc[t] = D16 ? r + (int)__ldcs(d + (k + t) * SLICE) : __ldcs(c + (k + t) * SLICE);
    }
    s0 = fma((double)vv[0], x[cc[0]], s0);
    s1 = fma((double)vv[1], x[cc[1]], s1);
    s0 = fma((double)vv[2], x[cc[2]], s0);
    s1 = fma((double)vv[3], x[cc[3]], s1);
  }
  for (; k < w; ++k)
  {
    const float vv = __ldcs(v + k * SLICE);
    const int cc = D16 ? r + (int)__ldcs(d + k * SLICE) : __ldcs(c + k * SLICE);
    s0 = fma((double)vv, x[cc], s0);
  }
  return s0 + s1;
}

template <bool D16>
__global__ void __launch_bounds__(ST)
k_spmv_sell(int n_rows, const long long* __restrict__ slice_ptr, const float* __restrict__ vals,
            const int16_t* __restrict__ dcol, const int32_t* __restrict__ cols, const double* __restrict__ x,
            double* __restrict__ y)
{
  const int row = blockIdx.x * blockDim.x + threadIdx.x;
  if ((row >> 5) >= (n_rows + SLICE - 1) / SLICE)
    return;
  const double s = sell_row<D16>(row, n_rows, slice_ptr, vals, dcol, cols, x);
  if (row < n_rows)
    y[row] = s;
}

template <bool D16, int MODE>
__global__ void __launch_bounds__(ST)
k_spmv_sell_cheb(int n_rows, const long long* __restrict__ slice_ptr, const float* __restrict__ vals,
                 const int16_t* __restrict__ dcol, const int32_t* __restrict__ cols,
                 const int32_t* __restrict__ off_diag, const int32_t* __restrict__ row_ptr,
                 const double* __restrict__ x, const ChebEp e)
{
  const int row = blockIdx.x * blockDim.x + threadIdx.x;
  if ((row >> 5) >= (n_rows + SLICE - 1) / SLICE)
    return;
  const double s = sell_row<D16>(row, n_rows, slice_ptr, vals, dcol, cols, x);
  if (row >= n_rows)
    return;
  if (off_diag && off_diag[row] < row_ptr[row + 1])
    e.scratch[row] = s;
  else
    cheb_row<MODE>(row, s, x, e);
}

template <bool ACCUM>
__global__ void __launch_bounds__(ST)
k_spmv_sell_rect(int n_rows, const long long* __restrict__ slice_ptr, const double* __restrict__ vals,
                 const int32_t* __restrict__ cols, const double* __restrict__ x, double* __restrict__ y)
{
  const int row = blockIdx.x * blockDim.x + threadIdx.x;
  const int s = row >> 5, lane = row & 31;
  if (row >= n_rows)
    return;
  const long long b = slice_ptr[s];
  const int w = (int)((slice_ptr[s + 1] - b) >> 5);
  const double* v = vals + b + lane;
  const int32_t* c = cols + b + lane;
  double s0 = 0.0, s1 = 0.0;
  int k = 0;
  for (; k + 2 <= w; k += 2)
  {
    const double v0 = __ldcs(v + k * SLICE), v1 = __ldcs(v + (k + 1) * SLICE);
    const int c0 = __ldcs(c + k * SLICE), c1 = __ldcs(c + (k + 1) * SLICE);
    s0 = fma(v0, x[c0], s0);
    s1 = fma(v1, x[c1], s1);
  }
  if (k < w)
    s0 = fma(__ldcs(v + k * SLICE), x[__ldcs(c + k * SLICE)], s0);
  y[row] = ACCUM ? y[row] + (s0 + s1) : s0 + s1;
}

__global__ void k_sell_widths(int n_rows, const int32_t* __restrict__ row_ptr, const int32_t* __restrict__ off_diag,
                              const int32_t* __restrict__ cols, long long* __restrict__ widths, int* __restrict__ overflow)
{
  const int row = blockIdx.x * blockDim.x + threadIdx.x;
  int len = 0;
  bool ovf = false;
  if (row < n_rows)
  {
    len = off_diag[row] - row_ptr[row];
    for (int j = row_ptr[row]; j < off_diag[row]; ++j)
    {
      const int dlt = cols[j] - row;
      ovf = ovf || dlt > 32767 || dlt < -32767;
    }
  }
#pragma unroll
  for (int o = 16; o > 0; o >>= 1)
    len = max(len, __shfl_xor_sync(0xffffffffu, len, o));
  if (__any_sync(0xffffffffu, ovf) && (threadIdx.x & 31) == 0)
    atomicOr(overflow, 1);
  if ((threadIdx.x & 31) == 0 && row < n_rows)
    widths[row >> 5] = (long long)len * SLICE;
}

__global__ void k_sell_fill(int n_rows, const int32_t* __restrict__ row_ptr, const int32_t* __restrict__ off_diag,
                            const int32_t* __restrict__ cols, const double* __restrict__ vals,
                            const long long* __restrict__ slice_ptr, float* __restrict__ v32, int16_t* __restrict__ d16,
                            int32_t* __restrict__ c32)
{
  const int row = blockIdx.x * blockDim.x + threadIdx.x;
  const int s = row >> 5, lane = row & 31;
  if (s >= (n_rows + SLICE - 1) / SLICE)
    return;
  const long long b = slice_ptr[s];
  const int w = (int)((slice_ptr[s + 1] - b) >> 5);
  const int r = row < n_rows ? row : n_rows - 1;
  const int beg = row < n_rows ? row_ptr[row] : 0, len = row < n_rows ? off_diag[row] - row_ptr[row] : 0;
  for (int k = 0; k < w; ++k)
  {
    const long long p = b + (long long)k * SLICE + lane;
    const bool ok = k < len;
    v32[p] = ok ? (float)vals[beg + k] : 0.f;
    const int col = ok ? cols[beg + k] : r;
    if (d16)
      d16[p] = (int16_t)(col - r);
    if (c32)
      c32[p] = col;
  }
}

template <int LANES, bool ACCUM>
__global__ void __launch_bounds__(ST)
k_spmv_rect(int n_rows, const double* __restrict__ vals, const int32_t* __restrict__ ptr,
            const int32_t* __restrict__ cols, const double* __restrict__ x, double* __restrict__ y)
{
  const int gt = blockIdx.x * blockDim.x + threadIdx.x;
  const int row = gt / LANES, lane = gt % LANES;
  double s = 0.0;
  if (row < n_rows)
  {
    const int e = ptr[row + 1];
    for (int j = ptr[row] + lane; j < e; j += LANES)
      s = fma(vals[j], x[cols[j]], s);
  }
#pragma unroll
  for (int o = LANES / 2; o > 0; o >>= 1)
    s += __shfl_xor_sync(0xffffffffu, s, o);
  if (row < n_rows && lane == 0)
    y[row] = ACCUM ? y[row] + s : s;
}
}

void spmv_sell_rect(pmgx_ctx* c, int n_rows, const long long* slice_ptr, const int32_t* cols, const double* vals,
                    const double* x, double* y, bool accumulate)
{
  if (n_rows <= 0)
    return;
  const int grid = (n_rows + ST - 1) / ST;
  if (accumulate)
    k_spmv_sell_rect<true><<<grid, ST, 0, c->stream>>>(n_rows, slice_ptr, vals, cols, x, y);
  else
    k_spmv_sell_rect<false><<<grid, ST, 0, c->stream>>>(n_rows, slice_ptr, vals, cols, x, y);
  check_launch("k_spmv_sell_rect");
  count_launch(c);
}

void spmv_rect(pmgx_ctx* c, int n_rows, const int32_t* row_ptr, const int32_t* cols, const double* vals,
               const double* x, double* y, bool accumulate, int lanes)
{
  if (n_rows <= 0)
    return;
  const int grid = (int)(((long long)n_rows * lanes + ST - 1) / ST);
  if (lanes == 32)
  {
    if (accumulate)
      k_spmv_rect<32, true><<<grid, ST, 0, c->stream>>>(n_rows, vals, row_ptr, cols, x, y);
    else
      k_spmv_rect<32, false><<<grid, ST, 0, c->stream>>>(n_rows, vals, row_ptr, cols, x, y);
  }
  else if (lanes == 4)
  {
    if (accumulate)
      k_spmv_rect<4, true><<<grid, ST, 0, c->stream>>>(n_rows, vals, row_ptr, cols, x, y);
    else
      k_spmv_rect<4, false><<<grid, ST, 0, c->stream>>>(n_rows, vals, row_ptr, cols, x, y);
  }
  else
  {
    if (accumulate)
      k_spmv_rect<8, true><<<grid, ST, 0, c->stream>>>(n_rows, vals, row_ptr, cols, x, y);
    else
      k_spmv_rect<8, false><<<grid, ST, 0, c->stream>>>(n_rows, vals, row_ptr, cols, x, y);
  }
  check_launch("k_spmv_rect");
  count_launch(c);
}

void CsrOperator::apply(double* x, double* y)
{
  cudaSetDevice(ctx->device);
  const int grid = (int)(((long long)n_owned * LPR + ST - 1) / ST);
  if (n_ghost > 0)
    vec::set(ctx, y + n_owned, n_ghost, 0.0);
  if (halo)
    halo_fwd_begin(halo, x);
  if (n_owned > 0)
  {
    k_spmv<false><<<grid, ST, 0, ctx->stream>>>(n_owned, values.p, row_ptr.p, off_diag.p, cols.p, x, y);
    check_launch("k_spmv");
    count_launch(ctx);
  }
  if (halo)
    halo_fwd_end(halo, x);
  if (n_ghost_rows > 0)
  {
    const int g2 = (int)(((long long)n_ghost_rows * LPR + ST - 1) / ST);
    k_spmv_ghost_rows<<<g2, ST, 0, ctx->stream>>>(n_ghost_rows, ghost_rows.p, values.p, off_diag.p, row_ptr.p, cols.p,
                                                  x, y);
    check_launch("k_spmv_ghost_rows");
    count_launch(ctx);
  }
}

bool CsrOperator::apply_cheb(double* in, const ChebEp& e)
{
  cudaSetDevice(ctx->device);
  PMGX_REQUIRE(n_ghost_rows == 0 || e.scratch, "apply_cheb: scratch vector missing");
  const int grid = (int)(((long long)n_owned * LPR + ST - 1) / ST);
  if (halo)
    halo_fwd_begin(halo, in);
  if (n_owned > 0)
    launch_spmv_cheb<double, false>(ctx, grid, n_owned, values.p, row_ptr.p, off_diag.p, row_ptr.p, nullptr, cols.p, in, e);
  if (halo)
    halo_fwd_end(halo, in);
  if (n_ghost_rows > 0)
    launch_ghost_rows_cheb(this, in, e);
  return true;
}

namespace
{
template <bool D16>
void launch_sell_cheb(const CsrOperatorLP* L, const double* x, const ChebEp& e)
{
  const CsrOperator* A = L->src;
  const int grid = (L->n_slices * SLICE + ST - 1) / ST;
  const int32_t* od = A->n_ghost_rows > 0 ? A->off_diag.p : nullptr;
#define PMGX_SC(M)                                                                                                     \
  k_spmv_sell_cheb<D16, M><<<grid, ST, 0, L->ctx->stream>>>(L->n_owned, L->slice_ptr.p, L->vals32.p, L->dcol16.p,       \
                                                            L->cols32.p, od, A->row_ptr.p, x, e)
  switch (e.mode)
  {
  case ChebEp::INIT: PMGX_SC(ChebEp::INIT); break;
  case ChebEp::STEP: PMGX_SC(ChebEp::STEP); break;
  case ChebEp::LAST: PMGX_SC(ChebEp::LAST); break;
  default: PMGX_SC(ChebEp::XONLY); break;
  }
#undef PMGX_SC
  check_launch("k_spmv_sell_cheb");
  count_launch(L->ctx);
}
}

void CsrOperatorLP::apply(double* x, double* y)
{
  cudaSetDevice(ctx->device);
  if (n_ghost > 0)
    vec::set(ctx, y + n_owned, n_ghost, 0.0);
  if (halo)
    halo_fwd_begin(halo, x);
  if (n_owned > 0)
  {
    const int grid = (n_slices * SLICE + ST - 1) / ST;
    if (d16)
      k_spmv_sell<true><<<grid, ST, 0, ctx->stream>>>(n_owned, slice_ptr.p, vals32.p, dcol16.p, nullptr, x, y);
    else
      k_spmv_sell<false><<<grid, ST, 0, ctx->stream>>>(n_owned, slice_ptr.p, vals32.p, nullptr, cols32.p, x, y);
    check_launch("k_spmv_sell");
    count_launch(ctx);
  }
  if (halo)
    halo_fwd_end(halo, x);
  if (src->n_ghost_rows > 0)
  {
    const int g2 = (int)(((long long)src->n_ghost_rows * LPR + ST - 1) / ST);
    k_spmv_ghost_rows<<<g2, ST, 0, ctx->stream>>>(src->n_ghost_rows, src->ghost_rows.p, src->values.p, src->off_diag.p,
                                                  src->row_ptr.p, src->cols.p, x, y);
    check_launch("k_spmv_ghost_rows");
    count_launch(ctx);
  }
}

bool CsrOperatorLP::apply_cheb(double* in, const ChebEp& e)
{
  cudaSetDevice(ctx->device);
  PMGX_REQUIRE(src->n_ghost_rows == 0 || e.scratch, "apply_cheb: scratch vector missing");
  if (halo)
    halo_fwd_begin(halo, in);
  if (n_owned > 0)
  {
    if (d16)
      launch_sell_cheb<true>(this, in, e);
    else
      launch_sell_cheb<false>(this, in, e);
  }
  if (halo)
    halo_fwd_end(halo, in);
  if (src->n_ghost_rows > 0)
    launch_ghost_rows_cheb(src, in, e);
  return true;
}

CsrOperatorLP* make_lp(CsrOperator* A)
{
  pmgx_ctx* c = A->ctx;
  std::unique_ptr<CsrOperatorLP> L(new CsrOperatorLP());
  L->ctx = c;
  L->kind = pmgx_operator::CSR;
  L->n_owned = A->n_owned;
  L->n_ghost = A->n_ghost;
  L->halo = A->halo;
  L->src = A;
  L->diag_inv.alloc((size_t)A->n_owned);
  if (A->n_owned > 0)
    PMGX_CUDA(cudaMemcpyAsync(L->diag_inv.p, A->diag_inv.p, (size_t)A->n_owned * sizeof(double), cudaMemcpyDeviceToDevice, c->stream));
  const int n = A->n_owned;
  L->n_slices = (n + SLICE - 1) / SLICE;
  L->slice_ptr.alloc((size_t)L->n_slices + 1);
  PMGX_CUDA(cudaMemsetAsync(L->slice_ptr.p, 0, ((size_t)L->n_slices + 1) * sizeof(long long), c->stream));
  DevBuf<int> ovf;
  ovf.alloc(1);
  PMGX_CUDA(cudaMemsetAsync(ovf.p, 0, sizeof(int), c->stream));
  long long total = 0;
  if (n > 0)
  {
    k_sell_widths<<<(n + ST - 1) / ST, ST, 0, c->stream>>>(n, A->row_ptr.p, A->off_diag.p, A->cols.p, L->slice_ptr.p + 1, ovf.p);
    check_launch("k_sell_widths");
    std::vector<long long> sp((size_t)L->n_slices + 1, 0);
    PMGX_CUDA(cudaMemcpyAsync(sp.data(), L->slice_ptr.p, sp.size() * sizeof(long long), cudaMemcpyDeviceToHost, c->stream));
    PMGX_CUDA(cudaStreamSynchronize(c->stream));
    for (size_t i = 1; i < sp.size(); ++i)
      sp[i] += sp[i - 1];
    total = sp.back();
    PMGX_CUDA(cudaMemcpyAsync(L->slice_ptr.p, sp.data(), sp.size() * sizeof(long long), cudaMemcpyHostToDevice, c->stream));
    PMGX_CUDA(cudaStreamSynchronize(c->stream));
  }
  int o = 0;
  PMGX_CUDA(cudaMemcpyAsync(&o, ovf.p, sizeof(int), cudaMemcpyDeviceToHost, c->stream));
  PMGX_CUDA(cudaStreamSynchronize(c->stream));
  L->d16 = o == 0;
  const size_t cap = (size_t)std::max<long long>(total, 1);
  L->vals32.alloc(cap);
  if (L->d16)
    L->dcol16.alloc(cap);
  else
    L->cols32.alloc(cap);
  if (n > 0)
  {
    k_sell_fill<<<(L->n_slices * SLICE + ST - 1) / ST, ST, 0, c->stream>>>(n, A->row_ptr.p, A->off_diag.p, A->cols.p, A->values.p,
                                                                         L->slice_ptr.p, L->vals32.p, L->dcol16.p, L->cols32.p);
    check_launch("k_sell_fill");
    PMGX_CUDA(cudaStreamSynchronize(c->stream));
  }
  return L.release();
}

void CsrOperator::finish_setup()
{
  n_ghost_rows = 0;
  if (n_owned > 0 && has_ghost_cols)
  {
    DevBuf<int32_t> count;
    count.alloc(1);
    ghost_rows.alloc((size_t)n_owned);
    PMGX_CUDA(cudaMemsetAsync(count.p, 0, sizeof(int32_t), ctx->stream));
    k_flag_ghost_rows<<<(n_owned + 255) / 256, 256, 0, ctx->stream>>>(n_owned, off_diag.p, row_ptr.p, count.p,
                                                                      ghost_rows.p);
    check_launch("k_flag_ghost_rows");
    PMGX_CUDA(cudaMemcpyAsync(&n_ghost_rows, count.p, sizeof(int32_t), cudaMemcpyDeviceToHost, ctx->stream));
    PMGX_CUDA(cudaStreamSynchronize(ctx->stream));
  }
  diag_inv.alloc((size_t)n_owned);
  if (n_owned > 0)
  {
    k_extract_diag_inv<<<(n_owned + 255) / 256, 256, 0, ctx->stream>>>(n_owned, values.p, row_ptr.p,
                                                                       cols.p, diag_inv.p);
    check_launch("k_extract_diag_inv");
    count_launch(ctx);
    PMGX_CUDA(cudaStreamSynchronize(ctx->stream));
  }
}
}

using pmgx::CsrOperator;

extern "C"
{
int pmgx_csr_create(pmgx_ctx* ctx, int n_rows, int n_ghost, const int32_t* row_ptr_h,
                    const int32_t* off_diag_offset_h, const int32_t* cols_h, const double* values_h,
                    pmgx_halo* halo, pmgx_operator** out)
{
  PMGX_API_BEGIN
  PMGX_REQUIRE(ctx && out && row_ptr_h, "csr_create: null argument");
  PMGX_REQUIRE(n_rows >= 0 && n_ghost >= 0, "csr_create: bad sizes");
  PMGX_CUDA(cudaSetDevice(ctx->device));
  const long long nnz = row_ptr_h[n_rows];
  PMGX_REQUIRE(row_ptr_h[0] == 0 && nnz >= 0, "csr_create: bad row_ptr");
  bool ghost_cols = false;
  for (int i = 0; i < n_rows; ++i)
  {
    PMGX_REQUIRE(row_ptr_h[i] <= off_diag_offset_h[i] && off_diag_offset_h[i] <= row_ptr_h[i + 1],
                 "csr_create: off_diag_offset outside its row");
    ghost_cols = ghost_cols || off_diag_offset_h[i] < row_ptr_h[i + 1];
  }
  for (long long j = 0; j < nnz; ++j)
    PMGX_REQUIRE(cols_h[j] >= 0 && cols_h[j] < n_rows + n_ghost, "csr_create: column out of range");
  std::unique_ptr<CsrOperator> A(new CsrOperator());
  A->ctx = ctx;
  A->kind = pmgx_operator::CSR;
  A->n_owned = n_rows;
  A->n_ghost = n_ghost;
  A->halo = halo;
  A->nnz = nnz;
  A->has_ghost_cols = ghost_cols;
  A->row_ptr.upload(row_ptr_h, (size_t)n_rows + 1, ctx->stream);
  A->off_diag.upload(off_diag_offset_h, (size_t)n_rows, ctx->stream);
  A->cols.upload(cols_h, (size_t)nnz, ctx->stream);
  A->values.upload(values_h, (size_t)nnz, ctx->stream);
  A->finish_setup();
  *out = A.release();
  PMGX_API_END
}

long long pmgx_csr_nnz(pmgx_operator* op)
{
  if (!op || op->kind != pmgx_operator::CSR)
    return -1;
  return static_cast<CsrOperator*>(op)->nnz;
}

int pmgx_csr_get(pmgx_operator* op, int32_t* row_ptr_h, int32_t* cols_h, double* values_h)
{
  PMGX_API_BEGIN
  PMGX_REQUIRE(op && op->kind == pmgx_operator::CSR, "csr_get: not a CSR operator");
  auto* A = static_cast<CsrOperator*>(op);
  PMGX_CUDA(cudaSetDevice(A->ctx->device));
  PMGX_CUDA(cudaStreamSynchronize(A->ctx->stream));
  if (row_ptr_h)
    PMGX_CUDA(cudaMemcpy(row_ptr_h, A->row_ptr.p, ((size_t)A->n_owned + 1) * sizeof(int32_t), cudaMemcpyDeviceToHost));
  if (cols_h && A->nnz > 0)
    PMGX_CUDA(cudaMemcpy(cols_h, A->cols.p, (size_t)A->nnz * sizeof(int32_t), cudaMemcpyDeviceToHost));
  if (values_h && A->nnz > 0)
    PMGX_CUDA(cudaMemcpy(values_h, A->values.p, (size_t)A->nnz * sizeof(double), cudaMemcpyDeviceToHost));
  PMGX_API_END
}
}
```

### pmg_dolfinx_b200/csrc/csr.hpp

```cpp
#pragma once
#include "operator.hpp"

namespace pmgx
{
struct CsrOperator : pmgx_operator
{
  long long nnz = 0;
  bool has_ghost_cols = false;
  DevBuf<int32_t> row_ptr;
  DevBuf<int32_t> off_diag;
  DevBuf<int32_t> cols;
  DevBuf<double> values;
  DevBuf<int32_t> ghost_rows;
  int n_ghost_rows = 0;
  void apply(double* x, double* y) override;
  bool supports_cheb_fusion() const override { return true; }
  bool apply_cheb(double* in, const ChebEp& e) override;
  void finish_setup();
};

struct CsrOperatorLP : pmgx_operator
{
  CsrOperator* src = nullptr;
  bool d16 = false;
  int n_slices = 0;
  DevBuf<long long> slice_ptr;
  DevBuf<float> vals32;
  DevBuf<int16_t> dcol16;
  DevBuf<int32_t> cols32;
  void apply(double* x, double* y) override;
  bool supports_cheb_fusion() const override { return true; }
  bool apply_cheb(double* in, const ChebEp& e) override;
};
CsrOperatorLP* make_lp(CsrOperator* A);
}
```

### pmg_dolfinx_b200/csrc/ctx.cu

```cuda
#include "common.hpp"

#include <cstdlib>
#include <cstring>

extern "C"
{
int pmgx_nccl_unique_id(void* id_h)
{
  PMGX_API_BEGIN
  static_assert(sizeof(ncclUniqueId) <= PMGX_NCCL_ID_BYTES, "ncclUniqueId too large");
  PMGX_REQUIRE(id_h != nullptr, "nccl_unique_id: null output");
  ncclUniqueId id;
  PMGX_NCCL(ncclGetUniqueId(&id));
  std::memset(id_h, 0, PMGX_NCCL_ID_BYTES);
  std::memcpy(id_h, &id, sizeof(id));
  PMGX_API_END
}

int pmgx_ctx_create(int device, int rank, int nranks, const void* nccl_id_h, pmgx_ctx** out)
{
  PMGX_API_BEGIN
  PMGX_REQUIRE(out != nullptr, "ctx_create: null output");
  PMGX_REQUIRE(nranks >= 1 && rank >= 0 && rank < nranks, "ctx_create: bad rank %d/%d", rank, nranks);
  PMGX_REQUIRE(nranks == 1 || nccl_id_h != nullptr, "ctx_create: nranks > 1 needs an NCCL id");
  int ndev = 0;
  PMGX_CUDA(cudaGetDeviceCount(&ndev));
  PMGX_REQUIRE(device >= 0 && device < ndev, "ctx_create: device %d not available (%d devices)", device, ndev);
  PMGX_CUDA(cudaSetDevice(device));
  cudaDeviceProp prop;
  PMGX_CUDA(cudaGetDeviceProperties(&prop, device));
  if (prop.major < 10)
  {
    pmgx::set_error("pmgx is built for sm_100a only; device %d is sm_%d%d", device, prop.major, prop.minor);
    return PMGX_ERR_UNSUPPORTED;
  }
  pmgx_ctx* c = new pmgx_ctx();
  c->device = device;
  c->rank = rank;
  c->nranks = nranks;
  c->num_sms = prop.multiProcessorCount;
  PMGX_CUDA(cudaStreamCreateWithFlags(&c->stream, cudaStreamNonBlocking));
  {
    int lo = 0, hi = 0;
    PMGX_CUDA(cudaDeviceGetStreamPriorityRange(&lo, &hi));
    PMGX_CUDA(cudaStreamCreateWithPriority(&c->comm_stream, cudaStreamNonBlocking, hi));
  }
  PMGX_CUDA(cudaMalloc(&c->d_scalars, 64 * sizeof(double)));
  PMGX_CUDA(cudaMemsetAsync(c->d_scalars, 0, 64 * sizeof(double), c->stream));
  PMGX_CUDA(cudaHostAlloc(&c->h_scalars, 64 * sizeof(double), cudaHostAllocMapped));
  PMGX_CUDA(cudaHostGetDevicePointer(&c->h_scalars_dev, c->h_scalars, 0));
  c->max_red_blocks = 8 * c->num_sms;
  PMGX_CUDA(cudaMalloc(&c->d_partials, (size_t)c->max_red_blocks * 4 * sizeof(double)));
  PMGX_CUDA(cudaMalloc(&c->d_counter, 16 * sizeof(unsigned int)));
  PMGX_CUDA(cudaMemsetAsync(c->d_counter, 0, 16 * sizeof(unsigned int), c->stream));
  PMGX_CUDA(cudaStreamSynchronize(c->stream));
  if (nranks > 1)
  {
    ncclUniqueId id;
    std::memcpy(&id, nccl_id_h, sizeof(id));
    PMGX_NCCL(ncclCommInitRank(&c->comm, nranks, id, rank));
    pmgx::p2p::ctx_setup(c);
  }
  *out = c;
  PMGX_API_END
}

int pmgx_ctx_destroy(pmgx_ctx* c)
{
  PMGX_API_BEGIN
  if (!c)
    return PMGX_OK;
  cudaSetDevice(c->device);
  cudaDeviceSynchronize();
  pmgx::p2p::ctx_teardown(c);
  if (c->comm)
    ncclCommDestroy(c->comm);
  cudaFree(c->d_scalars);
  cudaFreeHost(c->h_scalars);
  cudaFree(c->d_partials);
  cudaFree(c->d_counter);
  cudaStreamDestroy(c->stream);
  cudaStreamDestroy(c->comm_stream);
  delete c;
  PMGX_API_END
}

int pmgx_ctx_sync(pmgx_ctx* c)
{
  PMGX_API_BEGIN
  PMGX_REQUIRE(c, "ctx_sync: null ctx");
  PMGX_CUDA(cudaStreamSynchronize(c->comm_stream));
  PMGX_CUDA(cudaStreamSynchronize(c->stream));
  PMGX_API_END
}

int pmgx_ctx_profile(pmgx_ctx* c, int on)
{
  PMGX_API_BEGIN
  PMGX_REQUIRE(c, "ctx_profile: null ctx");
  c->profiling = on != 0;
  PMGX_API_END
}

int pmgx_ctx_profile_read(pmgx_ctx* c, int degree, double* ms_total_h, long long* launches_h)
{
  PMGX_API_BEGIN
  PMGX_REQUIRE(c && degree >= 1 && degree <= PMGX_MAX_DEGREE, "ctx_profile_read: bad arguments");
  PMGX_CUDA(cudaSetDevice(c->device));
  PMGX_CUDA(cudaStreamSynchronize(c->stream));
  double total = 0.0;
  for (auto& pr : c->prof[degree])
  {
    float ms = 0.f;
    PMGX_CUDA(cudaEventElapsedTime(&ms, pr.first, pr.second));
    total += ms;
    cudaEventDestroy(pr.first);
    cudaEventDestroy(pr.second);
  }
  if (ms_total_h)
    *ms_total_h = total;
  if (launches_h)
    *launches_h = (long long)c->prof[degree].size();
  c->prof[degree].clear();
  PMGX_API_END
}

void* pmgx_ctx_stream(pmgx_ctx* c) { return c ? (void*)c->stream : nullptr; }
int pmgx_ctx_rank(pmgx_ctx* c) { return c ? c->rank : -1; }
int pmgx_ctx_uses_p2p(pmgx_ctx* c) { return c && c->p2p ? 1 : 0; }
int pmgx_ctx_nranks(pmgx_ctx* c) { return c ? c->nranks : -1; }
long long pmgx_ctx_launch_count(pmgx_ctx* c) { return c ? c->launches : -1; }
}
```

### pmg_dolfinx_b200/csrc/solvers.cu

```cuda
#include "common.hpp"
#include "operator.hpp"
#include "reduce.cuh"
#include "solvers.hpp"

#include <cmath>
#include <cstdlib>
#include <cstring>

namespace pmgx
{
namespace
{
constexpr int FT = RED_THREADS;

inline int fused_grid(pmgx_ctx* c, long long n)
{
  long long b = (n + FT * 4 - 1) / (FT * 4);
  b = std::min<long long>(b, c->max_red_blocks);
  return (int)std::max<long long>(b, 1);
}

template <bool NORM>
__global__ void __launch_bounds__(FT)
k_cheb_init(const double* __restrict__ b, const double* __restrict__ q, const double* __restrict__ dinv,
            double* __restrict__ r, double* __restrict__ z, double* __restrict__ x, double c0,
            bool add_x, long long n, double* partials, unsigned int* counter, double* out)
{
  const long long nth = (long long)gridDim.x * blockDim.x;
  double s = 0.0;
  for (long long i = (long long)blockIdx.x * blockDim.x + threadIdx.x; i < n; i += nth)
  {
    const double rv = q ? q[i] * (-1.0) + b[i] : b[i];
    const double zv = (rv * dinv[i]) * c0;
    r[i] = rv;
    z[i] = zv;
    if (add_x)
      x[i] = q ? zv * 1.0 + x[i] : zv;
    if (NORM)
      s = fma(rv, rv, s);
  }
  if (NORM)
  {
    double v[1] = {s};
    grid_reduce<1>(v, partials, counter, out);
  }
}

template <bool NORM>
__global__ void __launch_bounds__(FT)
k_cheb_step(const double* __restrict__ q, const double* __restrict__ dinv, double* __restrict__ r,
            double* __restrict__ z, double* __restrict__ x, double c1, double c2, bool add_x, int defer,
            long long n, double* partials, unsigned int* counter, double* out)
{
  const long long nth = (long long)gridDim.x * blockDim.x;
  double s = 0.0;
  for (long long i = (long long)blockIdx.x * blockDim.x + threadIdx.x; i < n; i += nth)
  {
    const double rv = q[i] * (-1.0) + r[i];
    const double zo = z[i];
    const double zs = zo * c1;
    const double zv = (rv * dinv[i]) * c2 + zs;
    r[i] = rv;
    z[i] = zv;
    if (add_x)
    {
      const double xo = defer == 2 ? zo : (defer == 1 ? zo * 1.0 + x[i] : x[i]);
      x[i] = zv * 1.0 + xo;
    }
    if (NORM)
      s = fma(rv, rv, s);
  }
  if (NORM)
  {
    double v[1] = {s};
    grid_reduce<1>(v, partials, counter, out);
  }
}

template <bool NORM>
__global__ void __launch_bounds__(FT)
k_cheb_last(const double* __restrict__ q, double* __restrict__ r, long long n, double* partials,
            unsigned int* counter, double* out)
{
  const long long nth = (long long)gridDim.x * blockDim.x;
  double s = 0.0;
  for (long long i = (long long)blockIdx.x * blockDim.x + threadIdx.x; i < n; i += nth)
  {
    const double rv = q[i] * (-1.0) + r[i];
    r[i] = rv;
    if (NORM)
      s = fma(rv, rv, s);
  }
  if (NORM)
  {
    double v[1] = {s};
    grid_reduce<1>(v, partials, counter, out);
  }
}

template <int DUMMY>
__global__ void __launch_bounds__(FT)
k_cheb_step_xonly(const double* __restrict__ q, const double* __restrict__ dinv, const double* __restrict__ r,
                  const double* __restrict__ z, double* __restrict__ x, double c1, double c2, int defer,
                  long long n)
{
  const long long nth = (long long)gridDim.x * blockDim.x;
  for (long long i = (long long)blockIdx.x * blockDim.x + threadIdx.x; i < n; i += nth)
  {
    const double rv = q[i] * (-1.0) + r[i];
    const double zo = z[i];
    const double zs = zo * c1;
    const double zv = (rv * dinv[i]) * c2 + zs;
    const double xo = defer == 2 ? zo : (defer == 1 ? zo * 1.0 + x[i] : x[i]);
    x[i] = zv * 1.0 + xo;
  }
}

__global__ void __launch_bounds__(FT)
k_cg_init(const double* __restrict__ b, const double* __restrict__ y, const double* __restrict__ dinv,
          double* __restrict__ r, double* __restrict__ p, long long n, double* partials,
          unsigned int* counter, double* out)
{
  const long long nth = (long long)gridDim.x * blockDim.x;
  double s = 0.0;
  for (long long i = (long long)blockIdx.x * blockDim.x + threadIdx.x; i < n; i += nth)
  {
    const double rv = y[i] * (-1.0) + b[i];
    const double pv = rv * dinv[i];
    r[i] = rv;
    p[i] = pv;
    s = fma(pv, rv, s);
  }
  double v[1] = {s};
  grid_reduce<1>(v, partials, counter, out);
}

__global__ void __launch_bounds__(FT)
k_cg_update(double rnorm, const double* __restrict__ rnorm_dev, const double* __restrict__ pAp,
            const double* __restrict__ p, const double* __restrict__ dinv, double* __restrict__ x,
            double* __restrict__ r, double* __restrict__ y, long long n, double* partials,
            unsigned int* counter, double* out)
{
  if (rnorm_dev)
    rnorm = *rnorm_dev;
  const double alpha = rnorm / *pAp;
  const double nalpha = -alpha;
  const long long nth = (long long)gridDim.x * blockDim.x;
  double s = 0.0;
  for (long long i = (long long)blockIdx.x * blockDim.x + threadIdx.x; i < n; i += nth)
  {
    const double pv = p[i];
    x[i] = pv * alpha + x[i];
    const double rv = y[i] * nalpha + r[i];
    const double yv = rv * dinv[i];
    r[i] = rv;
    y[i] = yv;
    s = fma(rv, yv, s);
  }
  double v[1] = {s};
  grid_reduce<1>(v, partials, counter, out);
}

__global__ void __launch_bounds__(FT)
k_cgcg_init(const double* __restrict__ b, const double* __restrict__ q, const double* __restrict__ dinv,
            double* __restrict__ r, double* __restrict__ u, double* __restrict__ x, bool zero_x, long long n)
{
  const long long nth = (long long)gridDim.x * blockDim.x;
  for (long long i = (long long)blockIdx.x * blockDim.x + threadIdx.x; i < n; i += nth)
  {
    const double rv = q ? q[i] * (-1.0) + b[i] : b[i];
    r[i] = rv;
    if (dinv)
      u[i] = rv * dinv[i];
    if (zero_x)
      x[i] = 0.0;
  }
}

__global__ void __launch_bounds__(FT)
k_cgcg_update(const double* __restrict__ sc_cur, const double* __restrict__ sc_old,
              const double* __restrict__ alpha_old, double* __restrict__ alpha_out,
              double* __restrict__ gamma0_out, bool first,
              const double* __restrict__ dinv, const double* __restrict__ w, double* __restrict__ p,
              double* __restrict__ s, double* __restrict__ x, double* __restrict__ r, double* __restrict__ u,
              long long n)
{
  const double gamma = sc_cur[0], delta = sc_cur[1];
  double beta = first ? 0.0 : gamma / sc_old[0];
  double alpha = first ? gamma / delta : gamma / (delta - beta * gamma / *alpha_old);
  if (!(gamma > 0.0))
    alpha = 0.0, beta = 0.0;
  const long long nth = (long long)gridDim.x * blockDim.x;
  for (long long i = (long long)blockIdx.x * blockDim.x + threadIdx.x; i < n; i += nth)
  {
    const double pv = first ? u[i] : fma(beta, p[i], u[i]);
    const double sv = first ? w[i] : fma(beta, s[i], w[i]);
    p[i] = pv;
    s[i] = sv;
    x[i] = fma(alpha, pv, x[i]);
    const double rv = fma(-alpha, sv, r[i]);
    r[i] = rv;
    if (dinv)
      u[i] = rv * dinv[i];
  }
  if (blockIdx.x == 0 && threadIdx.x == 0)
  {
    *alpha_out = alpha;
    if (first)
      gamma0_out[0] = gamma;
  }
}

__global__ void __launch_bounds__(FT)
k_dot2(const double* __restrict__ r, const double* __restrict__ w, const double* __restrict__ u, long long n,
       double* partials, unsigned int* counter, double* out, const PeerReduce pr)
{
  const long long nth = (long long)gridDim.x * blockDim.x;
  double a = 0.0, b = 0.0;
  for (long long i = (long long)blockIdx.x * blockDim.x + threadIdx.x; i < n; i += nth)
  {
    const double uv = u[i];
    a = fma(r[i], uv, a);
    b = fma(w[i], uv, b);
  }
  double v[2] = {a, b};
  grid_reduce<2>(v, partials, counter, out, pr);
}

void check(const char* w) { check_launch(w); }
}
}


namespace pmgx
{

static void cheb_solve_fused(pmgx_cheb* s, pmgx_operator* A, double* x, const double* b, bool x_is_zero,
                             ChebResidual final_r)
{
  pmgx_ctx* c = s->ctx;
  const long long n = s->n_owned;
  const double lmax = s->eig_max;
  const size_t nt = (size_t)s->n_owned + s->n_ghost;
  if (s->z2.n != nt)
  {
    s->z2.alloc(nt);
    if (nt > 0)
      PMGX_CUDA(cudaMemsetAsync(s->z2.p, 0, nt * sizeof(double), c->stream));
  }
  double* zin = s->z.p;
  double* zout = s->z2.p;
  ChebEp e;
  e.b = b;
  e.r = s->r.p;
  e.x = x;
  e.dinv = A->diag_inv.p;
  e.scratch = s->q.p;
  e.c0 = 4.0 / (3.0 * lmax);
  if (x_is_zero)
  {
    k_cheb_init<false><<<fused_grid(c, n), FT, 0, c->stream>>>(b, nullptr, e.dinv, s->r.p, zin, x, e.c0, false, n,
                                                              c->d_partials, c->d_counter, c->d_scalars + 8);
    check("k_cheb_init");
    count_launch(c);
  }
  else
  {
    e.mode = ChebEp::INIT;
    e.z_out = zin;
    A->apply_cheb(x, e);
  }
  const int defer_mode = x_is_zero ? 2 : 1;
  for (int i = 1; i <= s->max_iter; ++i)
  {
    const bool last = i == s->max_iter;
    if (last && final_r == CHEB_R_NONE)
      break;
    if (last && final_r == CHEB_R_SPLIT)
    {
      A->apply(zin, s->q.p);
      break;
    }
    e.c1 = double(2 * i - 1) / double(2 * i + 3);
    e.c2 = double(8 * i + 4) / double(2 * i + 3) / lmax;
    e.defer = i == 1 ? defer_mode : 0;
    e.mode = last ? ChebEp::LAST : ((i + 1 == s->max_iter && final_r == CHEB_R_NONE) ? ChebEp::XONLY : ChebEp::STEP);
    e.z_out = zout;
    A->apply_cheb(zin, e);
    if (e.mode == ChebEp::STEP)
      std::swap(zin, zout);
  }
}

void cheb_solve(pmgx_cheb* s, pmgx_operator* A, double* x, const double* b, double* hist, bool x_is_zero,
                ChebResidual final_r)
{
  static const bool fuse = !(getenv("PMGX_CHEB_FUSE") && atoi(getenv("PMGX_CHEB_FUSE")) == 0);
  if (fuse && s->fuse && !hist && s->max_iter >= 2 && A->supports_cheb_fusion())
    return cheb_solve_fused(s, A, x, b, x_is_zero, final_r);
  pmgx_ctx* c = s->ctx;
  const long long n = s->n_owned;
  const double lmax = s->eig_max;
  const double* dinv = A->diag_inv.p;
  const int grid = fused_grid(c, n);
  if (hist)
    final_r = CHEB_R_FULL;
  if (s->max_iter == 0 && final_r == CHEB_R_SPLIT)
    final_r = CHEB_R_FULL;
  if (!x_is_zero)
    A->apply(x, s->q.p);
  const double* q0 = x_is_zero ? nullptr : s->q.p;
  const bool deferred = s->max_iter >= 2;
  const bool first_add = s->max_iter >= 1 && !deferred;
  const int defer_mode = !deferred ? 0 : (x_is_zero ? 2 : 1);
  const double c0 = 4.0 / (3.0 * lmax);
  if (hist)
    k_cheb_init<true><<<grid, FT, 0, c->stream>>>(b, q0, dinv, s->r.p, s->z.p, x, c0, first_add, n,
                                                  c->d_partials, c->d_counter, c->d_scalars + 8);
  else
    k_cheb_init<false><<<grid, FT, 0, c->stream>>>(b, q0, dinv, s->r.p, s->z.p, x, c0, first_add, n,
                                                   c->d_partials, c->d_counter, c->d_scalars + 8);
  check("k_cheb_init");
  count_launch(c);
  if (hist)
  {
    vec::allreduce_scalars(c, 8, 1, false);
    hist[0] = std::sqrt(vec::read_scalar(c, 8));
  }
  for (int i = 1; i <= s->max_iter; ++i)
  {
    const bool last = i == s->max_iter;
    if (last && final_r == CHEB_R_NONE)
      break;
    A->apply(s->z.p, s->q.p);
    if (last && final_r == CHEB_R_SPLIT)
      break;
    const double c1 = double(2 * i - 1) / double(2 * i + 3);
    const double c2 = double(8 * i + 4) / double(2 * i + 3) / lmax;
    if (last)
    {
      if (hist)
        k_cheb_last<true><<<grid, FT, 0, c->stream>>>(s->q.p, s->r.p, n, c->d_partials, c->d_counter,
                                                      c->d_scalars + 8);
      else
        k_cheb_last<false><<<grid, FT, 0, c->stream>>>(s->q.p, s->r.p, n, c->d_partials, c->d_counter,
                                                       c->d_scalars + 8);
      check("k_cheb_last");
    }
    else if (i + 1 == s->max_iter && final_r == CHEB_R_NONE)
    {
      k_cheb_step_xonly<0><<<grid, FT, 0, c->stream>>>(s->q.p, dinv, s->r.p, s->z.p, x, c1, c2,
                                                       i == 1 ? defer_mode : 0, n);
      check("k_cheb_step_xonly");
    }
    else
    {
      if (hist)
        k_cheb_step<true><<<grid, FT, 0, c->stream>>>(s->q.p, dinv, s->r.p, s->z.p, x, c1, c2, true,
                                                      i == 1 ? defer_mode : 0, n, c->d_partials, c->d_counter,
                                                      c->d_scalars + 8);
      else
        k_cheb_step<false><<<grid, FT, 0, c->stream>>>(s->q.p, dinv, s->r.p, s->z.p, x, c1, c2, true,
                                                       i == 1 ? defer_mode : 0, n, c->d_partials, c->d_counter,
                                                       c->d_scalars + 8);
      check("k_cheb_step");
    }
    count_launch(c);
    if (hist)
    {
      vec::allreduce_scalars(c, 8, 1, false);
      hist[i] = std::sqrt(vec::read_scalar(c, 8));
    }
  }
}
}


namespace pmgx
{
int cg_solve_pmg(pmgx_cg* s, pmgx_operator* A, double* x, const double* b)
{
  pmgx_ctx* c = s->ctx;
  const long long n = s->n_owned;
  const long long nt = (long long)s->n_owned + s->n_ghost;
  auto precond = [&](const double* r, double* z)
  {
    vec::set(c, z, nt, 0.0);
    const int rc = pmgx_vcycle_apply(s->precond, r, z, nullptr);
    if (rc != PMGX_OK)
      throw Error{rc};
  };
  s->history.clear();
  A->apply(x, s->y.p);
  vec::axpy(c, s->r.p, -1.0, s->y.p, b, n);
  precond(s->r.p, s->p.p);
  const double rnorm0 = vec::dot(c, s->p.p, s->r.p, n);
  s->rnorm0 = rnorm0;
  double rnorm = rnorm0;
  const double rtol2 = s->rtol * s->rtol;
  int k = 0;
  while (k < s->max_iter)
  {
    ++k;
    A->apply(s->p.p, s->y.p);
    const double alpha = rnorm / vec::dot(c, s->p.p, s->y.p, n);
    vec::axpy(c, x, alpha, s->p.p, x, n);
    vec::axpy(c, s->r.p, -alpha, s->y.p, s->r.p, n);
    precond(s->r.p, s->y.p);
    const double rnorm_new = vec::dot(c, s->r.p, s->y.p, n);
    const double beta = rnorm_new / rnorm;
    rnorm = rnorm_new;
    s->history.push_back(rnorm);
    if (rnorm / rnorm0 < rtol2)
      break;
    vec::axpy(c, s->p.p, beta, s->p.p, s->y.p, n);
    if (s->store)
    {
      s->alphas.push_back(alpha);
      s->betas.push_back(beta);
      s->residuals.push_back(rnorm);
    }
  }
  return k;
}

int cg_solve(pmgx_cg* s, pmgx_operator* A, double* x, const double* b)
{
  if (s->precond)
    return cg_solve_pmg(s, A, x, b);
  pmgx_ctx* c = s->ctx;
  const long long n = s->n_owned;
  const double* dinv = A->diag_inv.p;
  const int grid = fused_grid(c, n);
  s->history.clear();
  A->apply(x, s->y.p);
  k_cg_init<<<grid, FT, 0, c->stream>>>(b, s->y.p, dinv, s->r.p, s->p.p, n, c->d_partials,
                                        c->d_counter, c->d_scalars + 1);
  check("k_cg_init");
  count_launch(c);
  vec::allreduce_scalars(c, 1, 1, false);
  const double rnorm0 = vec::read_scalar(c, 1);
  s->rnorm0 = rnorm0;
  double rnorm = rnorm0;
  const double rtol2 = s->rtol * s->rtol;
  int k = 0;
  while (k < s->max_iter)
  {
    ++k;
    A->apply(s->p.p, s->y.p);
    vec::dot_device(c, s->p.p, s->y.p, n, 2);
    k_cg_update<<<grid, FT, 0, c->stream>>>(rnorm, nullptr, c->d_scalars + 2, s->p.p, dinv, x, s->r.p, s->y.p, n,
                                            c->d_partials, c->d_counter, c->d_scalars + 3);
    check("k_cg_update");
    count_launch(c);
    vec::allreduce_scalars(c, 3, 1, false);
    vec::publish_scalars(c, 2, 2);
    const double alpha = rnorm / c->h_scalars[2];
    const double rnorm_new = c->h_scalars[3];
    const double beta = rnorm_new / rnorm;
    rnorm = rnorm_new;
    s->history.push_back(rnorm);
    if (rnorm / rnorm0 < rtol2)
      break;
    vec::axpy(c, s->p.p, beta, s->p.p, s->y.p, n);
    if (s->store)
    {
      s->alphas.push_back(alpha);
      s->betas.push_back(beta);
      s->residuals.push_back(rnorm);
    }
  }
  return k;
}
}

namespace pmgx
{
int cgcg_solve(pmgx_coarse* co, double* x, const double* b, bool x_is_zero)
{
  pmgx_cg* s = co->cg;
  pmgx_operator* A = co->A;
  Precond* M = co->M;
  const int check_every = co->check_every;
  pmgx_ctx* c = s->ctx;
  const long long n = s->n_owned;
  const double* dinv = M ? nullptr : A->diag_inv.p;
  const int grid = fused_grid(c, n);
  const size_t nt = (size_t)s->n_owned + s->n_ghost;
  const size_t ntp = (nt + 15) & ~(size_t)15;
  if (s->slab.n != 5 * ntp)
  {
    s->slab.alloc(5 * ntp);
    if (nt > 0)
      PMGX_CUDA(cudaMemsetAsync(s->slab.p, 0, 5 * ntp * sizeof(double), c->stream));
    if (s->graph)
      cudaGraphExecDestroy(s->graph);
    if (s->graph_odd)
      cudaGraphExecDestroy(s->graph_odd);
    s->graph = s->graph_odd = nullptr;
  }
  double* const cr = s->slab.p;
  double* const w = s->slab.p + ntp;
  double* const cp = s->slab.p + 2 * ntp;
  double* const cu = s->slab.p + 3 * ntp;
  double* const cs = s->slab.p + 4 * ntp;
  double* sc = c->d_scalars + 16;
  double* al = c->d_scalars + 20;
  auto spmv_dots = [&](double* out2, int slot)
  {
    A->apply(cu, w);
    const PeerReduce pr = p2p::next_epoch(c);
    k_dot2<<<grid, FT, 0, c->stream>>>(cr, w, cu, n, c->d_partials, c->d_counter, out2, pr);
    check("k_dot2");
    count_launch(c);
    if (pr.nranks == 0)
      vec::allreduce_scalars(c, slot, 2, false);
  };
  if (!x_is_zero)
    A->apply(x, w);
  k_cgcg_init<<<grid, FT, 0, c->stream>>>(b, x_is_zero ? nullptr : w, dinv, cr, cu, x, x_is_zero, n);
  check("k_cgcg_init");
  count_launch(c);
  if (M)
    M->apply(cr, cu);
  spmv_dots(sc, 16);
  s->history.clear();
  const double rtol2 = s->rtol * s->rtol;
  double* g0 = c->d_scalars + 22;
  auto iterate = [&](int k)
  {
    const int cur = k & 1, nxt = cur ^ 1;
    k_cgcg_update<<<grid, FT, 0, c->stream>>>(sc + 2 * cur, sc + 2 * nxt, al + nxt, al + cur, g0, k == 0, dinv, w,
                                              cp, cs, x, cr, cu, n);
    check("k_cgcg_update");
    count_launch(c);
    if (k + 1 < s->max_iter)
    {
      if (M)
        M->apply(cr, cu);
      spmv_dots(sc + 2 * nxt, 16 + 2 * nxt);
    }
  };
  static const bool graphs_enabled = !(getenv("PMGX_COARSE_GRAPH") && atoi(getenv("PMGX_COARSE_GRAPH")) == 0);
  const bool block_ok = graphs_enabled && !s->graph_off && check_every >= 1;
  auto run_block = [&](int k0)
  {
    const void* key[3] = {A, x, reinterpret_cast<const void*>((size_t)check_every)};
    if ((s->graph || s->graph_odd) && (s->graph_key[0] != key[0] || s->graph_key[1] != key[1] || s->graph_key[2] != key[2]))
    {
      if (s->graph)
        cudaGraphExecDestroy(s->graph);
      if (s->graph_odd)
        cudaGraphExecDestroy(s->graph_odd);
      s->graph = s->graph_odd = nullptr;
    }
    cudaGraphExec_t& slot_graph = (k0 & 1) ? s->graph_odd : s->graph;
    if (!slot_graph)
    {
      const long long l0 = c->launches;
      cudaGraph_t g = nullptr;
      bool ok = cudaStreamBeginCapture(c->stream, cudaStreamCaptureModeRelaxed) == cudaSuccess;
      if (ok)
      {
        try
        {
          for (int k = k0; k < k0 + check_every; ++k)
            iterate(k);
        }
        catch (const Error&)
        {
          ok = false;
        }
        ok = (cudaStreamEndCapture(c->stream, &g) == cudaSuccess) && ok && g != nullptr;
      }
      if (ok)
        ok = cudaGraphInstantiate(&slot_graph, g, 0) == cudaSuccess;
      if (g)
        cudaGraphDestroy(g);
      s->graph_launches = (int)(c->launches - l0);
      c->launches = l0;
      if (!ok)
      {
        cudaGetLastError();
        slot_graph = nullptr;
        s->graph_off = true;
        for (int k = k0; k < k0 + check_every; ++k)
          iterate(k);
        return;
      }
      s->graph_key[0] = key[0], s->graph_key[1] = key[1], s->graph_key[2] = key[2];
    }
    PMGX_CUDA(cudaGraphLaunch(slot_graph, c->stream));
    count_launch(c, s->graph_launches);
  };
  int k = 0;
  co->last_converged = false;
  co->last_rel = 0.0;
  while (k < s->max_iter)
  {
    if (block_ok && k >= 2 && k % check_every == 0 && k + check_every < s->max_iter && !s->graph_off)
    {
      run_block(k);
      k += check_every;
    }
    else
    {
      iterate(k);
      ++k;
      if (k == s->max_iter)
        break;
    }
    const int nxt = k & 1;
    if (k % check_every == 0)
    {
      vec::publish_scalars(c, 16, 7);
      const double r = c->h_scalars[16 + 2 * nxt];
      s->rnorm0 = c->h_scalars[22];
      s->history.push_back(r);
      co->last_rel = s->rnorm0 > 0.0 ? std::sqrt(std::max(r, 0.0) / s->rnorm0) : 0.0;
      if (!(r > 0.0) || r / s->rnorm0 < rtol2)
      {
        co->last_converged = true;
        break;
      }
    }
  }
  return k;
}
}


struct pmgx_vcycle
{
  pmgx_ctx* ctx = nullptr;
  int n_levels = 0;
  int flags = 0;
  std::vector<pmgx_operator*> ops;
  std::vector<pmgx_cheb*> smoothers;
  std::vector<pmgx_interp*> interps;
  std::vector<const int8_t*> bc;
  pmgx_coarse* coarse = nullptr;
  std::vector<pmgx::DevBuf<double>> u, r, b;
  std::vector<double> diagnostics;
};

extern "C"
{
int pmgx_cheb_create(pmgx_ctx* ctx, int n_owned, int n_ghost, double eig_min, double eig_max, pmgx_cheb** out)
{
  PMGX_API_BEGIN
  PMGX_REQUIRE(ctx && out && n_owned >= 0 && n_ghost >= 0, "cheb_create: bad arguments");
  PMGX_REQUIRE(eig_max > 0.0, "cheb_create: eig_max must be positive");
  PMGX_CUDA(cudaSetDevice(ctx->device));
  std::unique_ptr<pmgx_cheb> s(new pmgx_cheb());
  s->ctx = ctx;
  s->n_owned = n_owned;
  s->n_ghost = n_ghost;
  s->eig_min = eig_min;
  s->eig_max = eig_max;
  const size_t nt = (size_t)n_owned + n_ghost;
  s->z.alloc(nt);
  s->q.alloc(nt);
  s->r.alloc(nt);
  if (nt > 0)
  {
    PMGX_CUDA(cudaMemsetAsync(s->z.p, 0, nt * sizeof(double), ctx->stream));
    PMGX_CUDA(cudaMemsetAsync(s->q.p, 0, nt * sizeof(double), ctx->stream));
    PMGX_CUDA(cudaMemsetAsync(s->r.p, 0, nt * sizeof(double), ctx->stream));
  }
  *out = s.release();
  PMGX_API_END
}
int pmgx_cheb_set_max_iterations(pmgx_cheb* s, int max_iter)
{
  PMGX_API_BEGIN
  PMGX_REQUIRE(s && max_iter >= 0, "cheb_set_max_iterations: bad arguments");
  s->max_iter = max_iter;
  PMGX_API_END
}
int pmgx_cheb_solve(pmgx_cheb* s, pmgx_operator* A, double* x, const double* b, double* resid_hist_h)
{
  PMGX_API_BEGIN
  PMGX_REQUIRE(s && A && x && b, "cheb_solve: null argument");
  PMGX_REQUIRE(A->n_owned == s->n_owned && A->n_ghost == s->n_ghost, "Incompatible vector sizes");
  PMGX_CUDA(cudaSetDevice(s->ctx->device));
  pmgx::cheb_solve(s, A, x, b, resid_hist_h, false, pmgx::CHEB_R_NONE);
  PMGX_API_END
}
int pmgx_cheb_residual(pmgx_cheb* s, pmgx_operator* A, double* x, const double* b, double* rnorm_h)
{
  PMGX_API_BEGIN
  PMGX_REQUIRE(s && A && x && b && rnorm_h, "cheb_residual: null argument");
  PMGX_REQUIRE(A->n_owned == s->n_owned && A->n_ghost == s->n_ghost, "Incompatible vector sizes");
  PMGX_CUDA(cudaSetDevice(s->ctx->device));
  A->apply(x, s->q.p);
  pmgx::vec::axpy(s->ctx, s->r.p, -1.0, s->q.p, b, s->n_owned);
  *rnorm_h = std::sqrt(pmgx::vec::dot(s->ctx, s->r.p, s->r.p, s->n_owned));
  PMGX_API_END
}
int pmgx_cheb_destroy(pmgx_cheb* s)
{
  PMGX_API_BEGIN
  if (s)
  {
    cudaSetDevice(s->ctx->device);
    cudaStreamSynchronize(s->ctx->stream);
    delete s;
  }
  PMGX_API_END
}

int pmgx_cg_create(pmgx_ctx* ctx, int n_owned, int n_ghost, pmgx_cg** out)
{
  PMGX_API_BEGIN
  PMGX_REQUIRE(ctx && out && n_owned >= 0 && n_ghost >= 0, "cg_create: bad arguments");
  PMGX_CUDA(cudaSetDevice(ctx->device));
  std::unique_ptr<pmgx_cg> s(new pmgx_cg());
  s->ctx = ctx;
  s->n_owned = n_owned;
  s->n_ghost = n_ghost;
  const size_t nt = (size_t)n_owned + n_ghost;
  s->r.alloc(nt);
  s->y.alloc(nt);
  s->p.alloc(nt);
  if (nt > 0)
  {
    PMGX_CUDA(cudaMemsetAsync(s->r.p, 0, nt * sizeof(double), ctx->stream));
    PMGX_CUDA(cudaMemsetAsync(s->y.p, 0, nt * sizeof(double), ctx->stream));
    PMGX_CUDA(cudaMemsetAsync(s->p.p, 0, nt * sizeof(double), ctx->stream));
  }
  *out = s.release();
  PMGX_API_END
}
int pmgx_cg_set_max_iterations(pmgx_cg* s, int max_iter)
{
  PMGX_API_BEGIN
  PMGX_REQUIRE(s && max_iter >= 0, "cg_set_max_iterations: bad arguments");
  s->max_iter = max_iter;
  s->alphas.reserve(max_iter);
  s->betas.reserve(max_iter);
  s->residuals.reserve(max_iter);
  PMGX_API_END
}
int pmgx_cg_set_tolerance(pmgx_cg* s, double rtol)
{
  PMGX_API_BEGIN
  PMGX_REQUIRE(s, "cg_set_tolerance: null solver");
  s->rtol = rtol;
  PMGX_API_END
}
int pmgx_cg_set_preconditioner(pmgx_cg* s, pmgx_vcycle* M)
{
  PMGX_API_BEGIN
  PMGX_REQUIRE(s, "cg_set_preconditioner: null solver");
  s->precond = M;
  PMGX_API_END
}
int pmgx_cg_store_coefficients(pmgx_cg* s, int on)
{
  PMGX_API_BEGIN
  PMGX_REQUIRE(s, "cg_store_coefficients: null solver");
  s->store = on != 0;
  PMGX_API_END
}
int pmgx_cg_solve(pmgx_cg* s, pmgx_operator* A, double* x, const double* b, int* iters_h)
{
  PMGX_API_BEGIN
  PMGX_REQUIRE(s && A && x && b, "cg_solve: null argument");
  PMGX_REQUIRE(A->n_owned == s->n_owned && A->n_ghost == s->n_ghost, "Incompatible vector sizes");
  PMGX_CUDA(cudaSetDevice(s->ctx->device));
  const int k = pmgx::cg_solve(s, A, x, b);
  if (iters_h)
    *iters_h = k;
  PMGX_API_END
}
int pmgx_cg_num_coefficients(pmgx_cg* s) { return s ? (int)s->alphas.size() : -1; }
int pmgx_cg_get_coefficients(pmgx_cg* s, double* alphas_h, double* betas_h, double* residuals_h)
{
  PMGX_API_BEGIN
  PMGX_REQUIRE(s, "cg_get_coefficients: null solver");
  for (size_t i = 0; i < s->alphas.size(); ++i)
  {
    if (alphas_h)
      alphas_h[i] = s->alphas[i];
    if (betas_h)
      betas_h[i] = s->betas[i];
    if (residuals_h)
      residuals_h[i] = s->residuals[i];
  }
  PMGX_API_END
}
int pmgx_cg_get_history(pmgx_cg* s, double* rnorm0_h, double* rnorms_h, int* n_h)
{
  PMGX_API_BEGIN
  PMGX_REQUIRE(s, "cg_get_history: null solver");
  if (rnorm0_h)
    *rnorm0_h = s->rnorm0;
  if (n_h)
    *n_h = (int)s->history.size();
  if (rnorms_h)
    for (size_t i = 0; i < s->history.size(); ++i)
      rnorms_h[i] = s->history[i];
  PMGX_API_END
}
int pmgx_cg_compute_eigenvalues(pmgx_cg* s, double* eig_h)
{
  PMGX_API_BEGIN
  PMGX_REQUIRE(s && eig_h, "cg_compute_eigenvalues: null argument");
  const int ne = (int)s->alphas.size();
  if (ne < 2)
  {
    pmgx::set_error("Insufficient data to compute eigenvalues");
    return PMGX_ERR_NUMERIC;
  }
  std::vector<double> d(ne, 0.0), e(ne, 0.0);
  for (int i = 0; i < ne; ++i)
    d[i] = 1.0 / s->alphas[i];
  for (int i = 0; i < ne - 1; ++i)
  {
    d[i + 1] += s->betas[i] / s->alphas[i];
    e[i] = std::sqrt(s->betas[i]) / s->alphas[i];
  }
  const int rc = pmgx_tqli(d.data(), e.data(), ne);
  if (rc != PMGX_OK)
    return rc;
  std::sort(d.begin(), d.end());
  for (int i = 0; i < ne; ++i)
    eig_h[i] = d[i];
  PMGX_API_END
}
int pmgx_cg_destroy(pmgx_cg* s)
{
  PMGX_API_BEGIN
  if (s)
  {
    cudaSetDevice(s->ctx->device);
    cudaStreamSynchronize(s->ctx->stream);
    if (s->graph)
      cudaGraphExecDestroy(s->graph);
    if (s->graph_odd)
      cudaGraphExecDestroy(s->graph_odd);
    delete s;
  }
  PMGX_API_END
}

int pmgx_coarse_create(pmgx_ctx* ctx, pmgx_operator* A, int max_iter, double rtol, pmgx_coarse** out)
{
  PMGX_API_BEGIN
  PMGX_REQUIRE(ctx && A && out && max_iter >= 0, "coarse_create: bad arguments");
  std::unique_ptr<pmgx_coarse> cs(new pmgx_coarse());
  cs->ctx = ctx;
  cs->A = A;
  int rc = pmgx_cg_create(ctx, A->n_owned, A->n_ghost, &cs->cg);
  if (rc != PMGX_OK)
    return rc;
  cs->cg->max_iter = max_iter;
  cs->cg->rtol = rtol;
  cs->cg->store = false;
  cs->cg->r.release();
  cs->cg->y.release();
  cs->cg->p.release();
  if (const char* e = getenv("PMGX_COARSE_CHECK_EVERY"))
    cs->check_every = std::max(atoi(e), 1);
  *out = cs.release();
  PMGX_API_END
}
int pmgx_coarse_solve(pmgx_coarse* cs, double* x, const double* b, int* iters_h)
{
  PMGX_API_BEGIN
  PMGX_REQUIRE(cs && x && b, "coarse_solve: null argument");
  PMGX_CUDA(cudaSetDevice(cs->ctx->device));
  const int k = pmgx::cgcg_solve(cs, x, b, false);
  cs->last_iters = k;
  if (iters_h)
    *iters_h = k;
  PMGX_API_END
}
int pmgx_coarse_last_iterations(pmgx_coarse* cs) { return cs ? cs->last_iters : -1; }
int pmgx_coarse_last_status(pmgx_coarse* cs, int* converged_h, double* rel_residual_h)
{
  PMGX_API_BEGIN
  PMGX_REQUIRE(cs, "coarse_last_status: null handle");
  if (converged_h)
    *converged_h = cs->last_converged ? 1 : 0;
  if (rel_residual_h)
    *rel_residual_h = cs->last_rel;
  PMGX_API_END
}

int pmgx_coarse_destroy(pmgx_coarse* cs)
{
  PMGX_API_BEGIN
  if (cs)
  {
    pmgx_cg_destroy(cs->cg);
    delete cs->M;
    delete cs;
  }
  PMGX_API_END
}

int pmgx_vcycle_create(pmgx_ctx* ctx, int n_levels, pmgx_operator** ops, pmgx_cheb** smoothers,
                       pmgx_interp** interps, const int8_t** bc_markers, pmgx_coarse* coarse, int flags,
                       pmgx_vcycle** out)
{
  PMGX_API_BEGIN
  PMGX_REQUIRE(ctx && out && n_levels >= 1 && ops && smoothers && bc_markers, "vcycle_create: bad arguments");
  PMGX_REQUIRE(n_levels == 1 || interps, "vcycle_create: interpolators missing");
  PMGX_CUDA(cudaSetDevice(ctx->device));
  std::unique_ptr<pmgx_vcycle> v(new pmgx_vcycle());
  v->ctx = ctx;
  v->n_levels = n_levels;
  v->flags = flags;
  v->coarse = coarse;
  v->u.resize(n_levels);
  v->r.resize(n_levels);
  v->b.resize(n_levels);
  for (int i = 0; i < n_levels; ++i)
  {
    PMGX_REQUIRE(ops[i] && smoothers[i] && bc_markers[i], "vcycle_create: null level %d", i);
    PMGX_REQUIRE(smoothers[i]->n_owned == ops[i]->n_owned, "Incompatible vector sizes");
    v->ops.push_back(ops[i]);
    v->smoothers.push_back(smoothers[i]);
    v->bc.push_back(bc_markers[i]);
    if (i < n_levels - 1)
    {
      PMGX_REQUIRE(interps[i], "vcycle_create: null interpolator %d", i);
      v->interps.push_back(interps[i]);
    }
    const size_t nt = (size_t)ops[i]->n_owned + ops[i]->n_ghost;
    const bool is_top = i == n_levels - 1 && n_levels > 1;
    for (auto* buf : {&v->u[i], &v->r[i], &v->b[i]})
    {
      if (is_top && buf != &v->r[i])
        continue;
      buf->alloc(nt);
      if (nt > 0)
        PMGX_CUDA(cudaMemsetAsync(buf->p, 0, nt * sizeof(double), ctx->stream));
    }
  }
  *out = v.release();
  PMGX_API_END
}

int pmgx_vcycle_apply(pmgx_vcycle* v, const double* b_in, double* u_inout, double* rnorm_h)
{
  PMGX_API_BEGIN
  PMGX_REQUIRE(v && b_in && u_inout, "vcycle_apply: null argument");
  pmgx_ctx* c = v->ctx;
  PMGX_CUDA(cudaSetDevice(c->device));
  const int nl = v->n_levels;
  const int top = nl - 1;
  const bool diag = (v->flags & PMGX_VC_DIAGNOSTICS) != 0;
  const bool literal_bc = (v->flags & PMGX_VC_LITERAL_REFERENCE_BC) != 0;
  const bool literal_seq = (v->flags & PMGX_VC_LITERAL_SEQUENCE) != 0;
  v->diagnostics.clear();
  namespace vec = pmgx::vec;
  std::vector<double*> U(nl);
  std::vector<const double*> B(nl);
  for (int i = 0; i < top; ++i)
    U[i] = v->u[i].p, B[i] = v->b[i].p;
  U[top] = u_inout;
  B[top] = b_in;
  auto residual = [&](int i, bool want_norm) -> double
  {
    pmgx_operator* A = v->ops[i];
    A->apply(U[i], v->r[i].p);
    vec::axpy(c, v->r[i].p, -1.0, v->r[i].p, B[i], A->n_owned);
    if (!want_norm)
      return 0.0;
    return std::sqrt(vec::dot(c, v->r[i].p, v->r[i].p, A->n_owned));
  };
  for (int i = 0; i < top; ++i)
    vec::set(c, U[i], (long long)v->ops[i]->n_owned + v->ops[i]->n_ghost, 0.0);

  for (int i = top; i > 0; --i)
  {
    if (diag)
      v->diagnostics.push_back(residual(i, true));
    const pmgx::ChebResidual want = literal_seq ? pmgx::CHEB_R_FULL : (diag ? pmgx::CHEB_R_FULL : pmgx::CHEB_R_SPLIT);
    pmgx::cheb_solve(v->smoothers[i], v->ops[i], U[i], B[i], nullptr, !literal_seq && i < top, want);
    double* rfine = v->r[i].p;
    const double* rsub = nullptr;
    if (literal_seq)
    {
      const double rn = residual(i, diag);
      if (diag)
        v->diagnostics.push_back(rn);
    }
    else
    {
      rfine = v->smoothers[i]->r.p;
      if (want == pmgx::CHEB_R_SPLIT && v->smoothers[i]->max_iter > 0)
        rsub = v->smoothers[i]->q.p;
      if (diag)
        v->diagnostics.push_back(std::sqrt(vec::dot(c, rfine, rfine, v->ops[i]->n_owned)));
    }
    pmgx::interp_restrict(v->interps[i - 1], rfine, rsub, v->b[i - 1].p);
    if (!literal_bc && i - 1 > 0)
      vec::mask_bc(c, v->b[i - 1].p, v->bc[i - 1], v->ops[i - 1]->n_owned);
  }
  if (nl > 1)
    vec::mask_bc(c, v->b[0].p, v->bc[0], v->ops[0]->n_owned);
  else
  {
    vec::copy(c, v->b[0].p, b_in, v->ops[0]->n_owned);
    vec::mask_bc(c, v->b[0].p, v->bc[0], v->ops[0]->n_owned);
    B[0] = v->b[0].p;
  }
  const pmgx::ChebResidual post = literal_seq ? pmgx::CHEB_R_FULL : pmgx::CHEB_R_NONE;
  if (v->coarse && nl > 1)
  {
    v->coarse->last_iters = pmgx::cgcg_solve(v->coarse, U[0], B[0], true);
  }
  else
    pmgx::cheb_solve(v->smoothers[0], v->ops[0], U[0], B[0], nullptr, !literal_seq && nl > 1, post);
  if (diag)
    v->diagnostics.push_back(residual(0, true));

  for (int i = 0; i < top; ++i)
  {
    pmgx::interp_prolong(v->interps[i], U[i], U[i + 1], true);
    if (diag)
      v->diagnostics.push_back(residual(i + 1, true));
    pmgx::cheb_solve(v->smoothers[i + 1], v->ops[i + 1], U[i + 1], B[i + 1], nullptr, false, post);
    if (diag && i + 1 < top)
      v->diagnostics.push_back(residual(i + 1, true));
  }
  if (rnorm_h || diag)
  {
    const double rn = residual(top, true);
    if (rnorm_h)
      *rnorm_h = rn;
    if (diag)
      v->diagnostics.push_back(rn);
  }
  PMGX_API_END
}

int pmgx_vcycle_get_diagnostics(pmgx_vcycle* v, double* out_h, int cap, int* n_h)
{
  PMGX_API_BEGIN
  PMGX_REQUIRE(v, "vcycle_get_diagnostics: null handle");
  const int n = (int)v->diagnostics.size();
  if (n_h)
    *n_h = n;
  if (out_h)
    for (int i = 0; i < n && i < cap; ++i)
      out_h[i] = v->diagnostics[i];
  PMGX_API_END
}

int pmgx_vcycle_destroy(pmgx_vcycle* v)
{
  PMGX_API_BEGIN
  if (v)
  {
    cudaSetDevice(v->ctx->device);
    cudaStreamSynchronize(v->ctx->stream);
    delete v;
  }
  PMGX_API_END
}
}
```

### pmg_dolfinx_b200/csrc/solvers.hpp

```cpp
#pragma once
#include "common.hpp"
#include "operator.hpp"

struct pmgx_cheb
{
  pmgx_ctx* ctx = nullptr;
  int n_owned = 0, n_ghost = 0;
  double eig_min = 0.0, eig_max = 1.0;
  int max_iter = 0;
  pmgx::DevBuf<double> z, q, r;
  pmgx::DevBuf<double> z2;
  bool fuse = true;
};

namespace pmgx
{
enum ChebResidual
{
  CHEB_R_NONE = 0,
  CHEB_R_FULL = 1,
  CHEB_R_SPLIT = 2
};
void cheb_solve(pmgx_cheb* s, pmgx_operator* A, double* x, const double* b, double* hist, bool x_is_zero = false,
                ChebResidual final_r = CHEB_R_FULL);

struct Precond
{
  virtual ~Precond() {}
  virtual void apply(const double* r, double* u) = 0;
};
}

struct pmgx_cg
{
  pmgx_ctx* ctx = nullptr;
  int n_owned = 0, n_ghost = 0;
  int max_iter = 0;
  double rtol = 0.0;
  bool store = false;
  pmgx_vcycle* precond = nullptr;
  pmgx::DevBuf<double> r, y, p;
  pmgx::DevBuf<double> slab;
  cudaGraphExec_t graph = nullptr, graph_odd = nullptr;
  const void* graph_key[3] = {nullptr, nullptr, nullptr};
  int graph_launches = 0;
  bool graph_off = false;
  std::vector<double> alphas, betas, residuals;
  std::vector<double> history;
  double rnorm0 = 0.0;
};

struct pmgx_coarse
{
  pmgx_ctx* ctx = nullptr;
  pmgx_operator* A = nullptr;
  pmgx_cg* cg = nullptr;
  pmgx::Precond* M = nullptr;
  int check_every = 8;
  int last_iters = 0;
  bool last_converged = false;
  double last_rel = 0.0;
};

namespace pmgx
{
int cgcg_solve(pmgx_coarse* cs, double* x, const double* b, bool x_is_zero);
void spmv_rect(pmgx_ctx* c, int n_rows, const int32_t* row_ptr, const int32_t* cols, const double* vals,
               const double* x, double* y, bool accumulate, int lanes);
void spmv_sell_rect(pmgx_ctx* c, int n_rows, const long long* slice_ptr, const int32_t* cols, const double* vals,
                    const double* x, double* y, bool accumulate);
}
```

Baseline: 5.437.

## Run coarse CG entirely on device with conditional while-graph and FP64 sliced-ELL operator

The coarse PCG solve is restructured into a CUDA graph with a conditional while node. A device kernel evaluates convergence and sets the loop condition, so the host no longer synchronises and reads residuals every check interval. Status and iteration counts are written to mapped host memory. The coarse operator used by CG also becomes an FP64 sliced-ELL copy of the CSR matrix for more coalesced SpMV, and a fused-smoother guard is added. The cost is extra device memory for the SELL values, plus a dependency on conditional graph nodes with a per-iteration synchronising fallback if capture fails.

```diff
diff --git a/include/pmgx.h b/include/pmgx.h
--- a/include/pmgx.h
+++ b/include/pmgx.h
@@ -147,6 +147,7 @@
 int pmgx_coarse_num_levels(pmgx_coarse* cs);
 int pmgx_coarse_level_info(pmgx_coarse* cs, int level, long long* out_h);
 int pmgx_coarse_apply_preconditioner(pmgx_coarse* cs, const double* r, double* u);
+int pmgx_coarse_apply_operator(pmgx_coarse* cs, double* x, double* y);
 int pmgx_coarse_destroy(pmgx_coarse* cs);
 
 typedef int (*pmgx_allgather_fn)(void* user, const void* mine, size_t bytes, void* all);
diff --git a/pmg_dolfinx_b200/api.py b/pmg_dolfinx_b200/api.py
--- a/pmg_dolfinx_b200/api.py
+++ b/pmg_dolfinx_b200/api.py
@@ -551,6 +551,9 @@
     def apply_preconditioner(self, r, u):
         check(lib.pmgx_coarse_apply_preconditioner(self.h, ptr(r.data), ptr(u.data)))
 
+    def apply_operator(self, x, y):
+        check(lib.pmgx_coarse_apply_operator(self.h, ptr(x.data), ptr(y.data)))
+
 
 class MultigridPreconditioner:
 
diff --git a/pmg_dolfinx_b200/csrc/amg.cu b/pmg_dolfinx_b200/csrc/amg.cu
--- a/pmg_dolfinx_b200/csrc/amg.cu
+++ b/pmg_dolfinx_b200/csrc/amg.cu
@@ -131,9 +131,12 @@
   int nu = 2;
   int gamma = 1;
   int gamma_from = 0;
+  pmgx_operator* A_pcg = nullptr;
 
   ~AmgPrecond() override
   {
+    if (A_pcg)
+      pmgx_operator_destroy(A_pcg);
     for (Lv& L : lv)
     {
       if (L.sm)
@@ -394,7 +397,7 @@
       D.sm->fuse = l >= fuse_from;
     }
     if (l == 0 && !last && use_lp)
-      D.A_lp = pmgx::make_lp(static_cast<pmgx::CsrOperator*>(D.A));
+      D.A_lp = pmgx::make_sell(static_cast<pmgx::CsrOperator*>(D.A), true);
     D.nnz_p = L.P.nnz();
     if (!last)
     {
@@ -415,16 +418,14 @@
         PMGX_CUDA(cudaMemsetAsync(D.b.p, 0, nt * sizeof(double), ctx->stream));
     }
   }
+  M->A_pcg = pmgx::make_sell(static_cast<pmgx::CsrOperator*>(M->lv[0].A), false);
   PMGX_CUDA(cudaStreamSynchronize(ctx->stream));
 
   pmgx_coarse* cs = nullptr;
-  const int rc = pmgx_coarse_create(ctx, M->lv[0].A, max_iter, rtol, &cs);
+  const int rc = pmgx_coarse_create(ctx, M->A_pcg, max_iter, rtol, &cs);
   if (rc != PMGX_OK)
     return rc;
   cs->M = M.release();
-  cs->check_every = 1;
-  if (const char* e = getenv("PMGX_COARSE_CHECK_EVERY"))
-    cs->check_every = std::max(atoi(e), 1);
   *out = cs;
   PMGX_API_END
 }
@@ -471,4 +472,13 @@
     pmgx::vec::pointwise_mult(cs->ctx, u, r, cs->A->diag_inv.p, cs->A->n_owned);
   PMGX_API_END
 }
-}
+
+int pmgx_coarse_apply_operator(pmgx_coarse* cs, double* x, double* y)
+{
+  PMGX_API_BEGIN
+  PMGX_REQUIRE(cs && x && y && x != y, "coarse_apply_operator: bad arguments");
+  PMGX_CUDA(cudaSetDevice(cs->ctx->device));
+  cs->A->apply(x, y);
+  PMGX_API_END
+}
+}
diff --git a/pmg_dolfinx_b200/csrc/common.hpp b/pmg_dolfinx_b200/csrc/common.hpp
--- a/pmg_dolfinx_b200/csrc/common.hpp
+++ b/pmg_dolfinx_b200/csrc/common.hpp
@@ -131,6 +131,8 @@
   unsigned long long* d_ar_epoch = nullptr;
   unsigned long long p2p_timeout_ns = 600ull * 1000000000ull;
   long long launches = 0;
+  unsigned long long* body_launches_h = nullptr;
+  unsigned long long* body_launches_dev = nullptr;
   bool profiling = false;
   std::vector<std::pair<cudaEvent_t, cudaEvent_t>> prof[PMGX_MAX_DEGREE + 1];
 };
diff --git a/pmg_dolfinx_b200/csrc/csr.cu b/pmg_dolfinx_b200/csrc/csr.cu
--- a/pmg_dolfinx_b200/csrc/csr.cu
+++ b/pmg_dolfinx_b200/csrc/csr.cu
@@ -231,15 +231,15 @@
 
 constexpr int SLICE = 32;
 
-template <bool D16>
+template <typename VT, bool D16>
 __device__ __forceinline__ double sell_row(int row, int n_rows, const long long* __restrict__ slice_ptr,
-                                           const float* __restrict__ vals, const int16_t* __restrict__ dcol,
+                                           const VT* __restrict__ vals, const int16_t* __restrict__ dcol,
                                            const int32_t* __restrict__ cols, const double* __restrict__ x)
 {
   const int s = row >> 5, lane = row & 31;
   const long long b = slice_ptr[s];
   const int w = (int)((slice_ptr[s + 1] - b) >> 5);
-  const float* v = vals + b + lane;
+  const VT* v = vals + b + lane;
   const int16_t* d = dcol + b + lane;
   const int32_t* c = cols + b + lane;
   const int r = row < n_rows ? row : n_rows - 1;
@@ -247,7 +247,7 @@
   int k = 0;
   for (; k + 4 <= w; k += 4)
   {
-    float vv[4];
+    VT vv[4];
     int cc[4];
 #pragma unroll
     for (int t = 0; t < 4; ++t)
@@ -262,23 +262,23 @@
   }
   for (; k < w; ++k)
   {
-    const float vv = __ldcs(v + k * SLICE);
+    const VT vv = __ldcs(v + k * SLICE);
     const int cc = D16 ? r + (int)__ldcs(d + k * SLICE) : __ldcs(c + k * SLICE);
     s0 = fma((double)vv, x[cc], s0);
   }
   return s0 + s1;
 }
 
-template <bool D16>
+template <typename VT, bool D16>
 __global__ void __launch_bounds__(ST)
-k_spmv_sell(int n_rows, const long long* __restrict__ slice_ptr, const float* __restrict__ vals,
+k_spmv_sell(int n_rows, const long long* __restrict__ slice_ptr, const VT* __restrict__ vals,
             const int16_t* __restrict__ dcol, const int32_t* __restrict__ cols, const double* __restrict__ x,
             double* __restrict__ y)
 {
   const int row = blockIdx.x * blockDim.x + threadIdx.x;
   if ((row >> 5) >= (n_rows + SLICE - 1) / SLICE)
     return;
-  const double s = sell_row<D16>(row, n_rows, slice_ptr, vals, dcol, cols, x);
+  const double s = sell_row<VT, D16>(row, n_rows, slice_ptr, vals, dcol, cols, x);
   if (row < n_rows)
     y[row] = s;
 }
@@ -293,7 +293,7 @@
   const int row = blockIdx.x * blockDim.x + threadIdx.x;
   if ((row >> 5) >= (n_rows + SLICE - 1) / SLICE)
     return;
-  const double s = sell_row<D16>(row, n_rows, slice_ptr, vals, dcol, cols, x);
+  const double s = sell_row<float, D16>(row, n_rows, slice_ptr, vals, dcol, cols, x);
   if (row >= n_rows)
     return;
   if (off_diag && off_diag[row] < row_ptr[row + 1])
@@ -355,8 +355,8 @@
 
 __global__ void k_sell_fill(int n_rows, const int32_t* __restrict__ row_ptr, const int32_t* __restrict__ off_diag,
                             const int32_t* __restrict__ cols, const double* __restrict__ vals,
-                            const long long* __restrict__ slice_ptr, float* __restrict__ v32, int16_t* __restrict__ d16,
-                            int32_t* __restrict__ c32)
+                            const long long* __restrict__ slice_ptr, float* __restrict__ v32, double* __restrict__ v64,
+                            int16_t* __restrict__ d16, int32_t* __restrict__ c32)
 {
   const int row = blockIdx.x * blockDim.x + threadIdx.x;
   const int s = row >> 5, lane = row & 31;
@@ -370,7 +370,10 @@
   {
     const long long p = b + (long long)k * SLICE + lane;
     const bool ok = k < len;
-    v32[p] = ok ? (float)vals[beg + k] : 0.f;
+    if (v32)
+      v32[p] = ok ? (float)vals[beg + k] : 0.f;
+    if (v64)
+      v64[p] = ok ? vals[beg + k] : 0.0;
     const int col = ok ? cols[beg + k] : r;
     if (d16)
       d16[p] = (int16_t)(col - r);
@@ -491,7 +494,7 @@
 namespace
 {
 template <bool D16>
-void launch_sell_cheb(const CsrOperatorLP* L, const double* x, const ChebEp& e)
+void launch_sell_cheb(const CsrOperatorSell* L, const double* x, const ChebEp& e)
 {
   const CsrOperator* A = L->src;
   const int grid = (L->n_slices * SLICE + ST - 1) / ST;
@@ -512,7 +515,7 @@
 }
 }
 
-void CsrOperatorLP::apply(double* x, double* y)
+void CsrOperatorSell::apply(double* x, double* y)
 {
   cudaSetDevice(ctx->device);
   if (n_ghost > 0)
@@ -522,10 +525,14 @@
   if (n_owned > 0)
   {
     const int grid = (n_slices * SLICE + ST - 1) / ST;
-    if (d16)
-      k_spmv_sell<true><<<grid, ST, 0, ctx->stream>>>(n_owned, slice_ptr.p, vals32.p, dcol16.p, nullptr, x, y);
+    if (vals64.p && d16)
+      k_spmv_sell<double, true><<<grid, ST, 0, ctx->stream>>>(n_owned, slice_ptr.p, vals64.p, dcol16.p, nullptr, x, y);
+    else if (vals64.p)
+      k_spmv_sell<double, false><<<grid, ST, 0, ctx->stream>>>(n_owned, slice_ptr.p, vals64.p, nullptr, cols32.p, x, y);
+    else if (d16)
+      k_spmv_sell<float, true><<<grid, ST, 0, ctx->stream>>>(n_owned, slice_ptr.p, vals32.p, dcol16.p, nullptr, x, y);
     else
-      k_spmv_sell<false><<<grid, ST, 0, ctx->stream>>>(n_owned, slice_ptr.p, vals32.p, nullptr, cols32.p, x, y);
+      k_spmv_sell<float, false><<<grid, ST, 0, ctx->stream>>>(n_owned, slice_ptr.p, vals32.p, nullptr, cols32.p, x, y);
     check_launch("k_spmv_sell");
     count_launch(ctx);
   }
@@ -541,9 +548,10 @@
   }
 }
 
-bool CsrOperatorLP::apply_cheb(double* in, const ChebEp& e)
+bool CsrOperatorSell::apply_cheb(double* in, const ChebEp& e)
 {
   cudaSetDevice(ctx->device);
+  PMGX_REQUIRE(supports_cheb_fusion(), "apply_cheb: the FP64 sliced-ELL twin has no fused smoother kernel");
   PMGX_REQUIRE(src->n_ghost_rows == 0 || e.scratch, "apply_cheb: scratch vector missing");
   if (halo)
     halo_fwd_begin(halo, in);
@@ -561,10 +569,10 @@
   return true;
 }
 
-CsrOperatorLP* make_lp(CsrOperator* A)
+CsrOperatorSell* make_sell(CsrOperator* A, bool fp32)
 {
   pmgx_ctx* c = A->ctx;
-  std::unique_ptr<CsrOperatorLP> L(new CsrOperatorLP());
+  std::unique_ptr<CsrOperatorSell> L(new CsrOperatorSell());
   L->ctx = c;
   L->kind = pmgx_operator::CSR;
   L->n_owned = A->n_owned;
@@ -600,7 +608,10 @@
   PMGX_CUDA(cudaStreamSynchronize(c->stream));
   L->d16 = o == 0;
   const size_t cap = (size_t)std::max<long long>(total, 1);
-  L->vals32.alloc(cap);
+  if (fp32)
+    L->vals32.alloc(cap);
+  else
+    L->vals64.alloc(cap);
   if (L->d16)
     L->dcol16.alloc(cap);
   else
@@ -608,7 +619,8 @@
   if (n > 0)
   {
     k_sell_fill<<<(L->n_slices * SLICE + ST - 1) / ST, ST, 0, c->stream>>>(n, A->row_ptr.p, A->off_diag.p, A->cols.p, A->values.p,
-                                                                         L->slice_ptr.p, L->vals32.p, L->dcol16.p, L->cols32.p);
+                                                                         L->slice_ptr.p, L->vals32.p, L->vals64.p, L->dcol16.p,
+                                                                         L->cols32.p);
     check_launch("k_sell_fill");
     PMGX_CUDA(cudaStreamSynchronize(c->stream));
   }
diff --git a/pmg_dolfinx_b200/csrc/csr.hpp b/pmg_dolfinx_b200/csrc/csr.hpp
--- a/pmg_dolfinx_b200/csrc/csr.hpp
+++ b/pmg_dolfinx_b200/csrc/csr.hpp
@@ -19,18 +19,19 @@
   void finish_setup();
 };
 
-struct CsrOperatorLP : pmgx_operator
+struct CsrOperatorSell : pmgx_operator
 {
   CsrOperator* src = nullptr;
   bool d16 = false;
   int n_slices = 0;
   DevBuf<long long> slice_ptr;
   DevBuf<float> vals32;
+  DevBuf<double> vals64;
   DevBuf<int16_t> dcol16;
   DevBuf<int32_t> cols32;
   void apply(double* x, double* y) override;
-  bool supports_cheb_fusion() const override { return true; }
+  bool supports_cheb_fusion() const override { return vals64.p == nullptr; }
   bool apply_cheb(double* in, const ChebEp& e) override;
 };
-CsrOperatorLP* make_lp(CsrOperator* A);
+CsrOperatorSell* make_sell(CsrOperator* A, bool fp32);
 }
diff --git a/pmg_dolfinx_b200/csrc/ctx.cu b/pmg_dolfinx_b200/csrc/ctx.cu
--- a/pmg_dolfinx_b200/csrc/ctx.cu
+++ b/pmg_dolfinx_b200/csrc/ctx.cu
@@ -49,6 +49,9 @@
   PMGX_CUDA(cudaMemsetAsync(c->d_scalars, 0, 64 * sizeof(double), c->stream));
   PMGX_CUDA(cudaHostAlloc(&c->h_scalars, 64 * sizeof(double), cudaHostAllocMapped));
   PMGX_CUDA(cudaHostGetDevicePointer(&c->h_scalars_dev, c->h_scalars, 0));
+  PMGX_CUDA(cudaHostAlloc(&c->body_launches_h, sizeof(unsigned long long), cudaHostAllocMapped));
+  PMGX_CUDA(cudaHostGetDevicePointer(&c->body_launches_dev, c->body_launches_h, 0));
+  *c->body_launches_h = 0;
   c->max_red_blocks = 8 * c->num_sms;
   PMGX_CUDA(cudaMalloc(&c->d_partials, (size_t)c->max_red_blocks * 4 * sizeof(double)));
   PMGX_CUDA(cudaMalloc(&c->d_counter, 16 * sizeof(unsigned int)));
@@ -77,6 +80,7 @@
     ncclCommDestroy(c->comm);
   cudaFree(c->d_scalars);
   cudaFreeHost(c->h_scalars);
+  cudaFreeHost(c->body_launches_h);
   cudaFree(c->d_partials);
   cudaFree(c->d_counter);
   cudaStreamDestroy(c->stream);
@@ -129,5 +133,10 @@
 int pmgx_ctx_rank(pmgx_ctx* c) { return c ? c->rank : -1; }
 int pmgx_ctx_uses_p2p(pmgx_ctx* c) { return c && c->p2p ? 1 : 0; }
 int pmgx_ctx_nranks(pmgx_ctx* c) { return c ? c->nranks : -1; }
-long long pmgx_ctx_launch_count(pmgx_ctx* c) { return c ? c->launches : -1; }
+long long pmgx_ctx_launch_count(pmgx_ctx* c)
+{
+  if (!c || cudaSetDevice(c->device) != cudaSuccess || cudaStreamSynchronize(c->stream) != cudaSuccess)
+    return -1;
+  return c->launches + (long long)*c->body_launches_h;
 }
+}
diff --git a/pmg_dolfinx_b200/csrc/solvers.cu b/pmg_dolfinx_b200/csrc/solvers.cu
--- a/pmg_dolfinx_b200/csrc/solvers.cu
+++ b/pmg_dolfinx_b200/csrc/solvers.cu
@@ -163,8 +163,14 @@
 
 __global__ void __launch_bounds__(FT)
 k_cgcg_init(const double* __restrict__ b, const double* __restrict__ q, const double* __restrict__ dinv,
-            double* __restrict__ r, double* __restrict__ u, double* __restrict__ x, bool zero_x, long long n)
-{
+            double* __restrict__ r, double* __restrict__ u, double* __restrict__ x, bool zero_x, long long n,
+            double* __restrict__ k_dev, double* __restrict__ status)
+{
+  if (blockIdx.x == 0 && threadIdx.x == 0)
+  {
+    *k_dev = 0.0;
+    status[0] = status[1] = status[2] = status[3] = 0.0;
+  }
   const long long nth = (long long)gridDim.x * blockDim.x;
   for (long long i = (long long)blockIdx.x * blockDim.x + threadIdx.x; i < n; i += nth)
   {
@@ -209,6 +215,41 @@
     if (first)
       gamma0_out[0] = gamma;
   }
+}
+
+__global__ void k_cgcg_test(double* __restrict__ sc, double* __restrict__ al, const double* __restrict__ g0,
+                            double* __restrict__ k_dev, int max_iter, double rtol2, double* __restrict__ status,
+                            cudaGraphConditionalHandle cond, bool use_cond, unsigned long long* body_launches,
+                            int n_body)
+{
+  if (n_body > 0)
+    *body_launches += n_body;
+  const double r = sc[2], d = sc[3];
+  sc[2] = sc[0];
+  sc[3] = sc[1];
+  sc[0] = r;
+  sc[1] = d;
+  const double a = al[0];
+  al[0] = al[1];
+  al[1] = a;
+  const int k = (int)*k_dev + 1;
+  *k_dev = k;
+  bool stop = k >= max_iter;
+  if (!stop)
+  {
+    const double r0 = *g0;
+    status[2] = r0 > 0.0 ? sqrt((r < 0.0 ? 0.0 : r) / r0) : 0.0;
+    if (!(r > 0.0) || r / r0 < rtol2)
+    {
+      stop = true;
+      status[1] = 1.0;
+    }
+  }
+  status[0] = k;
+  status[3] = stop ? 1.0 : 0.0;
+  __threadfence_system();
+  if (use_cond)
+    cudaGraphSetConditional(cond, stop ? 0u : 1u);
 }
 
 __global__ void __launch_bounds__(FT)
@@ -476,12 +517,11 @@
 
 namespace pmgx
 {
-int cgcg_solve(pmgx_coarse* co, double* x, const double* b, bool x_is_zero)
+void cgcg_solve(pmgx_coarse* co, double* x, const double* b, bool x_is_zero)
 {
   pmgx_cg* s = co->cg;
   pmgx_operator* A = co->A;
   Precond* M = co->M;
-  const int check_every = co->check_every;
   pmgx_ctx* c = s->ctx;
   const long long n = s->n_owned;
   const double* dinv = M ? nullptr : A->diag_inv.p;
@@ -495,9 +535,7 @@
       PMGX_CUDA(cudaMemsetAsync(s->slab.p, 0, 5 * ntp * sizeof(double), c->stream));
     if (s->graph)
       cudaGraphExecDestroy(s->graph);
-    if (s->graph_odd)
-      cudaGraphExecDestroy(s->graph_odd);
-    s->graph = s->graph_odd = nullptr;
+    s->graph = nullptr;
   }
   double* const cr = s->slab.p;
   double* const w = s->slab.p + ntp;
@@ -506,126 +544,126 @@
   double* const cs = s->slab.p + 4 * ntp;
   double* sc = c->d_scalars + 16;
   double* al = c->d_scalars + 20;
-  auto spmv_dots = [&](double* out2, int slot)
+  double* g0 = c->d_scalars + 22;
+  double* k_dev = c->d_scalars + 23;
+  const double rtol2 = s->rtol * s->rtol;
+  auto spmv_dots = [&](int slot)
   {
     A->apply(cu, w);
     const PeerReduce pr = p2p::next_epoch(c);
-    k_dot2<<<grid, FT, 0, c->stream>>>(cr, w, cu, n, c->d_partials, c->d_counter, out2, pr);
+    k_dot2<<<grid, FT, 0, c->stream>>>(cr, w, cu, n, c->d_partials, c->d_counter, c->d_scalars + slot, pr);
     check("k_dot2");
     count_launch(c);
     if (pr.nranks == 0)
       vec::allreduce_scalars(c, slot, 2, false);
   };
-  if (!x_is_zero)
-    A->apply(x, w);
-  k_cgcg_init<<<grid, FT, 0, c->stream>>>(b, x_is_zero ? nullptr : w, dinv, cr, cu, x, x_is_zero, n);
-  check("k_cgcg_init");
-  count_launch(c);
-  if (M)
-    M->apply(cr, cu);
-  spmv_dots(sc, 16);
-  s->history.clear();
-  const double rtol2 = s->rtol * s->rtol;
-  double* g0 = c->d_scalars + 22;
-  auto iterate = [&](int k)
-  {
-    const int cur = k & 1, nxt = cur ^ 1;
-    k_cgcg_update<<<grid, FT, 0, c->stream>>>(sc + 2 * cur, sc + 2 * nxt, al + nxt, al + cur, g0, k == 0, dinv, w,
-                                              cp, cs, x, cr, cu, n);
+  auto prologue = [&]()
+  {
+    if (!x_is_zero)
+      A->apply(x, w);
+    k_cgcg_init<<<grid, FT, 0, c->stream>>>(b, x_is_zero ? nullptr : w, dinv, cr, cu, x, x_is_zero, n, k_dev,
+                                            co->status_dev);
+    check("k_cgcg_init");
+    count_launch(c);
+    if (M)
+      M->apply(cr, cu);
+    spmv_dots(16);
+  };
+  auto iterate = [&](bool first, cudaGraphConditionalHandle cond, bool use_cond, bool in_body)
+  {
+    const long long l0 = c->launches;
+    k_cgcg_update<<<grid, FT, 0, c->stream>>>(sc, sc + 2, al + 1, al, g0, first, dinv, w, cp, cs, x, cr, cu, n);
     check("k_cgcg_update");
     count_launch(c);
-    if (k + 1 < s->max_iter)
-    {
-      if (M)
-        M->apply(cr, cu);
-      spmv_dots(sc + 2 * nxt, 16 + 2 * nxt);
-    }
+    if (M)
+      M->apply(cr, cu);
+    spmv_dots(18);
+    const int n_body = in_body ? (int)(c->launches - l0) + 1 : 0;
+    k_cgcg_test<<<1, 1, 0, c->stream>>>(sc, al, g0, k_dev, s->max_iter, rtol2, co->status_dev, cond, use_cond,
+                                        c->body_launches_dev, n_body);
+    check("k_cgcg_test");
+    count_launch(c);
   };
   static const bool graphs_enabled = !(getenv("PMGX_COARSE_GRAPH") && atoi(getenv("PMGX_COARSE_GRAPH")) == 0);
-  const bool block_ok = graphs_enabled && !s->graph_off && check_every >= 1;
-  auto run_block = [&](int k0)
-  {
-    const void* key[3] = {A, x, reinterpret_cast<const void*>((size_t)check_every)};
-    if ((s->graph || s->graph_odd) && (s->graph_key[0] != key[0] || s->graph_key[1] != key[1] || s->graph_key[2] != key[2]))
-    {
-      if (s->graph)
-        cudaGraphExecDestroy(s->graph);
-      if (s->graph_odd)
-        cudaGraphExecDestroy(s->graph_odd);
-      s->graph = s->graph_odd = nullptr;
-    }
-    cudaGraphExec_t& slot_graph = (k0 & 1) ? s->graph_odd : s->graph;
-    if (!slot_graph)
-    {
-      const long long l0 = c->launches;
-      cudaGraph_t g = nullptr;
-      bool ok = cudaStreamBeginCapture(c->stream, cudaStreamCaptureModeRelaxed) == cudaSuccess;
-      if (ok)
+  const void* key[3] = {x, b, reinterpret_cast<const void*>((size_t)x_is_zero)};
+  if (s->graph && (s->graph_key[0] != key[0] || s->graph_key[1] != key[1] || s->graph_key[2] != key[2]))
+  {
+    cudaGraphExecDestroy(s->graph);
+    s->graph = nullptr;
+  }
+  if (graphs_enabled && !s->graph_off && !s->graph && s->max_iter > 0)
+  {
+    const long long l0 = c->launches;
+    cudaGraph_t g = nullptr, body = nullptr;
+    cudaGraphConditionalHandle cond = 0;
+    bool ok = cudaGraphCreate(&g, 0) == cudaSuccess &&
+              cudaGraphConditionalHandleCreate(&cond, g, 1, cudaGraphCondAssignDefault) == cudaSuccess &&
+              cudaStreamBeginCaptureToGraph(c->stream, g, nullptr, nullptr, 0, cudaStreamCaptureModeRelaxed) == cudaSuccess;
+    if (ok)
+    {
+      try
       {
-        try
+        prologue();
+        iterate(true, cond, true, false);
+        cudaStreamCaptureStatus st;
+        const cudaGraphNode_t* deps = nullptr;
+        size_t n_deps = 0;
+        ok = cudaStreamGetCaptureInfo(c->stream, &st, nullptr, nullptr, &deps, &n_deps) == cudaSuccess;
+        cudaGraphNodeParams cp_ = {};
+        cp_.type = cudaGraphNodeTypeConditional;
+        cp_.conditional.handle = cond;
+        cp_.conditional.type = cudaGraphCondTypeWhile;
+        cp_.conditional.size = 1;
+        cudaGraphNode_t node = nullptr;
+        ok = ok && cudaGraphAddNode(&node, g, deps, n_deps, &cp_) == cudaSuccess;
+        body = ok ? cp_.conditional.phGraph_out[0] : nullptr;
+        cudaGraph_t g2 = nullptr;
+        ok = cudaStreamEndCapture(c->stream, &g2) == cudaSuccess && ok;
+        s->graph_launches = (int)(c->launches - l0);
+        ok = ok && cudaStreamBeginCaptureToGraph(c->stream, body, nullptr, nullptr, 0, cudaStreamCaptureModeRelaxed) == cudaSuccess;
+        if (ok)
         {
-          for (int k = k0; k < k0 + check_every; ++k)
-            iterate(k);
+          iterate(false, cond, true, true);
+          cudaGraph_t g3 = nullptr;
+          ok = cudaStreamEndCapture(c->stream, &g3) == cudaSuccess;
         }
-        catch (const Error&)
-        {
-          ok = false;
-        }
-        ok = (cudaStreamEndCapture(c->stream, &g) == cudaSuccess) && ok && g != nullptr;
       }
-      if (ok)
-        ok = cudaGraphInstantiate(&slot_graph, g, 0) == cudaSuccess;
-      if (g)
-        cudaGraphDestroy(g);
-      s->graph_launches = (int)(c->launches - l0);
-      c->launches = l0;
-      if (!ok)
+      catch (const Error&)
       {
-        cudaGetLastError();
-        slot_graph = nullptr;
-        s->graph_off = true;
-        for (int k = k0; k < k0 + check_every; ++k)
-          iterate(k);
-        return;
+        ok = false;
+        cudaGraph_t gx = nullptr;
+        cudaStreamCaptureStatus st;
+        if (cudaStreamIsCapturing(c->stream, &st) == cudaSuccess && st != cudaStreamCaptureStatusNone)
+          cudaStreamEndCapture(c->stream, &gx);
       }
+    }
+    ok = ok && cudaGraphInstantiate(&s->graph, g, 0) == cudaSuccess;
+    if (g)
+      cudaGraphDestroy(g);
+    c->launches = l0;
+    if (!ok)
+    {
+      cudaGetLastError();
+      s->graph = nullptr;
+      s->graph_off = true;
+    }
+    else
       s->graph_key[0] = key[0], s->graph_key[1] = key[1], s->graph_key[2] = key[2];
-    }
-    PMGX_CUDA(cudaGraphLaunch(slot_graph, c->stream));
+  }
+  if (s->graph)
+  {
+    PMGX_CUDA(cudaGraphLaunch(s->graph, c->stream));
     count_launch(c, s->graph_launches);
-  };
-  int k = 0;
-  co->last_converged = false;
-  co->last_rel = 0.0;
-  while (k < s->max_iter)
-  {
-    if (block_ok && k >= 2 && k % check_every == 0 && k + check_every < s->max_iter && !s->graph_off)
-    {
-      run_block(k);
-      k += check_every;
-    }
-    else
-    {
-      iterate(k);
-      ++k;
-      if (k == s->max_iter)
-        break;
-    }
-    const int nxt = k & 1;
-    if (k % check_every == 0)
-    {
-      vec::publish_scalars(c, 16, 7);
-      const double r = c->h_scalars[16 + 2 * nxt];
-      s->rnorm0 = c->h_scalars[22];
-      s->history.push_back(r);
-      co->last_rel = s->rnorm0 > 0.0 ? std::sqrt(std::max(r, 0.0) / s->rnorm0) : 0.0;
-      if (!(r > 0.0) || r / s->rnorm0 < rtol2)
-      {
-        co->last_converged = true;
-        break;
-      }
-    }
-  }
-  return k;
+    return;
+  }
+  prologue();
+  for (int k = 0; k < s->max_iter; ++k)
+  {
+    iterate(k == 0, 0, false, false);
+    PMGX_CUDA(cudaStreamSynchronize(c->stream));
+    if (co->status[3] != 0.0)
+      break;
+  }
 }
 }
 
@@ -838,8 +876,6 @@
     cudaStreamSynchronize(s->ctx->stream);
     if (s->graph)
       cudaGraphExecDestroy(s->graph);
-    if (s->graph_odd)
-      cudaGraphExecDestroy(s->graph_odd);
     delete s;
   }
   PMGX_API_END
@@ -861,8 +897,9 @@
   cs->cg->r.release();
   cs->cg->y.release();
   cs->cg->p.release();
-  if (const char* e = getenv("PMGX_COARSE_CHECK_EVERY"))
-    cs->check_every = std::max(atoi(e), 1);
+  PMGX_CUDA(cudaHostAlloc(&cs->status, 4 * sizeof(double), cudaHostAllocMapped));
+  PMGX_CUDA(cudaHostGetDevicePointer(&cs->status_dev, cs->status, 0));
+  std::memset(cs->status, 0, 4 * sizeof(double));
   *out = cs.release();
   PMGX_API_END
 }
@@ -871,21 +908,30 @@
   PMGX_API_BEGIN
   PMGX_REQUIRE(cs && x && b, "coarse_solve: null argument");
   PMGX_CUDA(cudaSetDevice(cs->ctx->device));
-  const int k = pmgx::cgcg_solve(cs, x, b, false);
-  cs->last_iters = k;
+  pmgx::cgcg_solve(cs, x, b, false);
   if (iters_h)
-    *iters_h = k;
-  PMGX_API_END
-}
-int pmgx_coarse_last_iterations(pmgx_coarse* cs) { return cs ? cs->last_iters : -1; }
+  {
+    PMGX_CUDA(cudaStreamSynchronize(cs->ctx->stream));
+    *iters_h = (int)cs->status[0];
+  }
+  PMGX_API_END
+}
+int pmgx_coarse_last_iterations(pmgx_coarse* cs)
+{
+  if (!cs || cudaSetDevice(cs->ctx->device) != cudaSuccess || cudaStreamSynchronize(cs->ctx->stream) != cudaSuccess)
+    return -1;
+  return (int)cs->status[0];
+}
 int pmgx_coarse_last_status(pmgx_coarse* cs, int* converged_h, double* rel_residual_h)
 {
   PMGX_API_BEGIN
   PMGX_REQUIRE(cs, "coarse_last_status: null handle");
+  PMGX_CUDA(cudaSetDevice(cs->ctx->device));
+  PMGX_CUDA(cudaStreamSynchronize(cs->ctx->stream));
   if (converged_h)
-    *converged_h = cs->last_converged ? 1 : 0;
+    *converged_h = cs->status[1] != 0.0 ? 1 : 0;
   if (rel_residual_h)
-    *rel_residual_h = cs->last_rel;
+    *rel_residual_h = cs->status[2];
   PMGX_API_END
 }
 
@@ -896,6 +942,8 @@
   {
     pmgx_cg_destroy(cs->cg);
     delete cs->M;
+    if (cs->status)
+      cudaFreeHost(cs->status);
     delete cs;
   }
   PMGX_API_END
@@ -1012,7 +1060,7 @@
   const pmgx::ChebResidual post = literal_seq ? pmgx::CHEB_R_FULL : pmgx::CHEB_R_NONE;
   if (v->coarse && nl > 1)
   {
-    v->coarse->last_iters = pmgx::cgcg_solve(v->coarse, U[0], B[0], true);
+    pmgx::cgcg_solve(v->coarse, U[0], B[0], true);
   }
   else
     pmgx::cheb_solve(v->smoothers[0], v->ops[0], U[0], B[0], nullptr, !literal_seq && nl > 1, post);
diff --git a/pmg_dolfinx_b200/csrc/solvers.hpp b/pmg_dolfinx_b200/csrc/solvers.hpp
--- a/pmg_dolfinx_b200/csrc/solvers.hpp
+++ b/pmg_dolfinx_b200/csrc/solvers.hpp
@@ -41,7 +41,7 @@
   pmgx_vcycle* precond = nullptr;
   pmgx::DevBuf<double> r, y, p;
   pmgx::DevBuf<double> slab;
-  cudaGraphExec_t graph = nullptr, graph_odd = nullptr;
+  cudaGraphExec_t graph = nullptr;
   const void* graph_key[3] = {nullptr, nullptr, nullptr};
   int graph_launches = 0;
   bool graph_off = false;
@@ -56,15 +56,13 @@
   pmgx_operator* A = nullptr;
   pmgx_cg* cg = nullptr;
   pmgx::Precond* M = nullptr;
-  int check_every = 8;
-  int last_iters = 0;
-  bool last_converged = false;
-  double last_rel = 0.0;
+  double* status = nullptr;
+  double* status_dev = nullptr;
 };
 
 namespace pmgx
 {
-int cgcg_solve(pmgx_coarse* cs, double* x, const double* b, bool x_is_zero);
+void cgcg_solve(pmgx_coarse* cs, double* x, const double* b, bool x_is_zero);
 void spmv_rect(pmgx_ctx* c, int n_rows, const int32_t* row_ptr, const int32_t* cols, const double* vals,
                const double* x, double* y, bool accumulate, int lanes);
 void spmv_sell_rect(pmgx_ctx* c, int n_rows, const long long* slice_ptr, const int32_t* cols, const double* vals,
```

Result: faster. 5.631 (median of 6 runs) (+3.6%).
